# adrelino/mv-lm-icp

Measured on AMD Instinct MI355X. Metric: ICP iterations/sec (NN+Jacobian+LM), higher is better.
Workload: dtype f64; 1 GPU; cfg4: multiview 32 views x 200k pts, point-to-plane, SophusSE3 (E=62); views=32, pts_per_view=200000, edges=62, parallelism=single GPU, nn=auto

## Files before the change

include/mvicp.h:

```cpp
#ifndef MVICP_H
#define MVICP_H

#include <stddef.h>
#include <stdint.h>

#ifdef __cplusplus
extern "C" {
#endif

typedef struct mvicp_ctx mvicp_ctx;

enum mvicp_status {
  MVICP_OK = 0,
  MVICP_ERR_ARG = -1,
  MVICP_ERR_HIP = -2,
  MVICP_ERR_STATE = -3,
  MVICP_ERR_COMM = -4,
  MVICP_ERR_NUMERIC = -5,
  MVICP_ERR_INTERNAL = -6
};

enum mvicp_param {
  MVICP_PARAM_EIGEN_QUATERNION = 0,
  MVICP_PARAM_ANGLE_AXIS = 1,
// ... 33 lines not shown
  long long n, kept;
  int q_exp;
  int has_normals;
  unsigned long long s1, s2_hi, s2_lo;
  double T;
  double threshold;
} mvicp_outlier_stats;
long long mvicp_outlier_filter(mvicp_ctx* ctx, int frame, int k, double std_ratio, double radius, mvicp_outlier_stats* stats);
int mvicp_outlier_fetch(mvicp_ctx* ctx, long long cap_kept, double* xyz, double* nrm, int* idx, long long cap_n, double* mdist, double* kd2);
int mvicp_outlier_threshold(long long n, unsigned long long s1, unsigned long long s2_hi, unsigned long long s2_lo, double std_ratio, double* T);

long long mvicp_knn_search(mvicp_ctx* ctx, int frame, const double* queries, long long m, int k, double radius);
int mvicp_knn_fetch(mvicp_ctx* ctx, long long cap_rows, long long cap_entries, int* cnt, long long* off, int* idx, double* d2);

long long mvicp_fpfh(mvicp_ctx* ctx, int frame, double radius, int max_nn);
int mvicp_fpfh_fetch(mvicp_ctx* ctx, long long cap_rows, double* desc, int* used);

long long mvicp_iss_keypoints(mvicp_ctx* ctx, int frame, double salient_radius, double non_max_radius, double gamma21, double gamma32,
                              int min_neighbors);
int mvicp_iss_fetch(mvicp_ctx* ctx, long long cap_keys, int* idx, double* xyz, double* nrm, long long cap_n, double* saliency, int* cnt_salient,
                    int* cnt_nms);

long long mvicp_estimate_normals(mvicp_ctx* ctx, int frame, int max_nn, double radius, const double* viewpoint);
int mvicp_normals_fetch(mvicp_ctx* ctx, long long cap_rows, double* nrm, double* curvature, int* used);
int mvicp_normals_adopt(mvicp_ctx* ctx);

long long mvicp_fit_normals(mvicp_ctx* ctx, int frame, int max_nn, double radius, const double* viewpoint, int degree);
int mvicp_normals_fit_fetch(mvicp_ctx* ctx, long long cap_rows, unsigned char* fitted);

typedef enum { MVICP_ORIENT_ANCHOR = 0, MVICP_ORIENT_VIEWPOINT = 1, MVICP_ORIENT_DIRECTION = 2 } mvicp_orient_mode;
long long mvicp_orient_normals(mvicp_ctx* ctx, int frame, int source, int k, double radius, int mode, const double* ref3);
int mvicp_orient_fetch(mvicp_ctx* ctx, long long cap_rows, double* nrm, unsigned char* flip, int* comp);
int mvicp_orient_adopt(mvicp_ctx* ctx);

int mvicp_normal_agreement(mvicp_ctx* ctx, const double* poses, int* pos, int* neg);
int mvicp_signs_from_agreement(int n_frames, int n_edges, const int* src, const int* dst, const int* pos, const int* neg, int min_count,
                               unsigned char* flip, int* component);
int mvicp_negate_normals(mvicp_ctx* ctx, int frame);

long long mvicp_feature_match(mvicp_ctx* ctx, const double* a, long long m, const double* b, long long n, int dim);
int mvicp_feature_match_fetch(mvicp_ctx* ctx, long long cap_m, long long cap_n, int* fwd_idx, double* fwd_d2, int* bwd_idx, double* bwd_d2);

long long mvicp_match_pairs(long long m, long long n, const int* fwd_idx, const double* fwd_d2, const int* bwd_idx, int mutual, double ratio,
                            int* pairs);

typedef struct mvicp_consensus_result {
  int best, count, accepted, reserved;
  double pose[16];
} mvicp_consensus_result;
int mvicp_consensus(mvicp_ctx* ctx, const double* p, const double* q, long long n_pairs, long long hypotheses, unsigned long long seed,
                    double tau, double edge_sim, mvicp_consensus_result* result);
int mvicp_consensus_fetch(mvicp_ctx* ctx, long long cap_h, int* count, long long cap_c, unsigned char* flags);

typedef struct mvicp_coarse_edge {
  int pairs, best, count, accepted;
  double pose[16];
} mvicp_coarse_edge;
long long mvicp_coarse_pairs(mvicp_ctx* ctx, const double* desc, const double* xyz, const long long* offsets, int n_sets, int dim, int n_edges,
                             const int* src, const int* dst, const unsigned long long* seeds, int mutual, double ratio, long long hypotheses,
                             double tau, double edge_sim, mvicp_coarse_edge* results);
int mvicp_coarse_pairs_fetch(mvicp_ctx* ctx, int edge, long long cap_pairs, int* pairs, unsigned char* flags);

int mvicp_poses_from_pairs(int n_frames, int n_edges, const int* src, const int* dst, const int* count, const double* pose, int min_count,
                           int root, const double* root_pose, double* poses_out, int* parent, int* parent_edge, int* component);

int mvicp_cache_allowance(const double* pose_src_old, const double* pose_dst_old, const double* pose_src, const double* pose_dst,
                          double max_norm, double* out);

int mvicp_graph_from_overlap(int n_frames, const int* samples, const int* hits, const long long* sumq, int knn, double min_fraction,
                             int skip_frame0, int cap, int* src, int* dst, int* n_components);

int mvicp_set_shard(mvicp_ctx* ctx, int rank, int world);
int mvicp_edge_owner(int n_edges, const int* n_src, int world, int* owner);
int mvicp_comm_unique_id(const char* librccl_path, void* unique_id_128);
int mvicp_comm_init(mvicp_ctx* ctx, const char* librccl_path, const void* unique_id_128, int rank, int world);
int mvicp_comm_nranks(mvicp_ctx* ctx);

typedef int (*mvicp_allreduce_fn)(void* user, double* host_buf, size_t n);
int mvicp_comm_set_callback(mvicp_ctx* ctx, mvicp_allreduce_fn fn, void* user);

int mvicp_correspond(mvicp_ctx* ctx, const double* poses, const unsigned char* fixed, float thresh, int nn_method,
                     int* counts, float* weights);
int mvicp_reset_history(mvicp_ctx* ctx);
int mvicp_get_correspondences(mvicp_ctx* ctx, int edge, int cap, int* first, int* second, double* dist);
typedef struct mvicp_corr { int first; int second; double dist; } mvicp_corr;
int mvicp_map_correspondences(mvicp_ctx* ctx, const mvicp_corr** triples, const long long** offsets);
int mvicp_map_correspondences_async(mvicp_ctx* ctx, const mvicp_corr** triples, const long long** offsets);
int mvicp_wait_correspondences(mvicp_ctx* ctx, int edge);
int mvicp_correspondence_epochs(mvicp_ctx* ctx, const unsigned long long** epochs);
int mvicp_set_correspondences(mvicp_ctx* ctx, int edge, int n, const int* first, const int* second, float weight);

int mvicp_nn_query(mvicp_ctx* ctx, int frame, const double* queries, int n, int nn_method, int* idx, double* d2);

#define MVICP_EDGE_BLOCK 91
int mvicp_linearize(mvicp_ctx* ctx, const double* poses, int point_to_plane, int robust, double* out);
int mvicp_linearize_pair(mvicp_ctx* ctx, const double* poses_a, const double* poses_b, int point_to_plane, int robust, double* out_a, double* out_b);

typedef enum { MVICP_METRIC_POINT = 0, MVICP_METRIC_PLANE = 1, MVICP_METRIC_SYMMETRIC = 2 } mvicp_metric;
int mvicp_linearize_metric(mvicp_ctx* ctx, const double* poses, int metric, int robust, double* out);

int mvicp_linearize_gicp(mvicp_ctx* ctx, const double* poses, double epsilon, int robust, double* out);

typedef struct mvicp_summary {
  double initial_cost, final_cost;
  int iterations;
  int successful_steps;
  int termination;
  int evaluations;
} mvicp_summary;
int mvicp_optimize(mvicp_ctx* ctx, double* poses, unsigned char* fixed, int param, int point_to_plane, int robust,
                   int max_iterations , mvicp_summary* summary);
int mvicp_optimize_metric(mvicp_ctx* ctx, double* poses, unsigned char* fixed, int param, int metric, int robust,
                          int max_iterations, mvicp_summary* summary);
int mvicp_optimize_gicp(mvicp_ctx* ctx, double* poses, unsigned char* fixed, int param, double epsilon, int robust,
                        int max_iterations, mvicp_summary* summary);

typedef int (*mvicp_eval_fn)(void* user, const double* poses, double* blocks);
int mvicp_lm_solve(int n_frames, int n_edges, const int* src, const int* dst, double* poses, unsigned char* fixed, int param,
                   int max_iterations, mvicp_eval_fn eval, void* user, mvicp_summary* summary);

int mvicp_closedform_point_to_point(const double* src, const double* dst, int n, double* pose_out);
int mvicp_closedform_point_to_plane(const double* src, const double* dst, const double* nor, int n, double* pose_out);

int mvicp_set_option(mvicp_ctx* ctx, const char* name, double value);
int mvicp_nn_census(mvicp_ctx* ctx, double* out5);
int mvicp_nn_census_ex(mvicp_ctx* ctx, double* out, int cap);
const char* mvicp_last_nn_launch(mvicp_ctx* ctx);

int mvicp_profile_enable(mvicp_ctx* ctx, int on);
int mvicp_profile_reset(mvicp_ctx* ctx);
int mvicp_profile_get(mvicp_ctx* ctx, const char* kernel, double* total_ms, long long* launches, double* alg_bytes);
int mvicp_profile_get_ex(mvicp_ctx* ctx, const char* kernel, double* out, int cap);
void* mvicp_stream(mvicp_ctx* ctx);
int mvicp_sync(mvicp_ctx* ctx);

#ifdef __cplusplus
}
#endif
#endif
```

mv-lm-icp_amd/csrc/api.cpp:

```cpp
#include <algorithm>
#include <cmath>
#include <cstdlib>
#include <cstring>
#include <ctime>
#include <chrono>
#include <condition_variable>
#include <exception>
#include <limits>
#include <mutex>
#include <new>
#include <thread>

#include "common.h"
#include "comm.h"
#include "nn_tie.h"
#include "../host/se3.h"

namespace mvicp {

static thread_local char g_err[1024] = "";

void set_error(const char* fmt, ...) {
  va_list ap;
  va_start(ap, fmt);
// ... 44 lines not shown
    MV_HIP(hipMalloc((void**)&c->d_scratch, c->scratch_bytes));
  }
  void* d = c->d_scratch + c->scratch_used;
  MV_HIP(hipMemcpyAsync(d, src, bytes, hipMemcpyHostToDevice, c->stream));
  MV_HIP(hipStreamSynchronize(c->stream));
  c->scratch_used += aligned;
  *dptr = d;
  return MVICP_OK;
}

ProfScope::ProfScope(mvicp_ctx* ctx, const char* nm, double bytes) : c(ctx), name(nm), on(ctx->profile) {
  if (on && ctx->profile_level >= 2 && ((std::strncmp(nm, "nn_", 3) != 0 && std::strncmp(nm, "linearize", 9) != 0 && std::strcmp(nm, "comm") != 0) ||
                                        std::strcmp(nm, "nn_tie") == 0)) on = false;
  if (!on) return;
  ProfEntry& pe = c->prof[name];
  auto get = [&]() {
    hipEvent_t ev = nullptr;
    if (!pe.pool.empty()) { ev = pe.pool.back(); pe.pool.pop_back(); }
    else if (hipEventCreate(&ev) != hipSuccess) ev = nullptr;
    return ev;
  };
  a = get(); b = get();
  pe.bytes += bytes;
  if (std::strncmp(nm, "nn_", 3) == 0) { pe.survey_bytes += bytes; pe.queries += bytes / 36.0; }
  pe.launches += 1;
  if (a) (void)hipEventRecord(a, c->stream);
}
ProfScope::~ProfScope() {
  if (!on) return;
  if (b) (void)hipEventRecord(b, c->stream);
  if (a && b) c->prof[name].pending.push_back(std::make_pair(a, b));
}
static double now_ms() {
  timespec ts;
  clock_gettime(CLOCK_MONOTONIC, &ts);
  return ts.tv_sec * 1e3 + ts.tv_nsec * 1e-6;
}
HostScope::HostScope(mvicp_ctx* ctx, const char* nm) : c(ctx), name(nm), t0(0.0), on(ctx->profile) { if (on) t0 = now_ms(); }
HostScope::~HostScope() {
  if (!on) return;
  ProfEntry& pe = c->prof[name];
  pe.ms += now_ms() - t0;
  pe.launches += 1;
}
void prof_collect_lazy(mvicp_ctx* c) {
  for (auto& kv : c->prof) if (kv.second.pending.size() > 256) { prof_collect(c); return; }
}
void prof_collect(mvicp_ctx* c) {
  for (auto& kv : c->prof) {
    ProfEntry& pe = kv.second;
    for (auto& pr : pe.pending) {
      float ms = 0.f;
      if (hipEventSynchronize(pr.second) == hipSuccess && hipEventElapsedTime(&ms, pr.first, pr.second) == hipSuccess) pe.ms += ms;
      pe.pool.push_back(pr.first);
      pe.pool.push_back(pr.second);
    }
    pe.pending.clear();
  }
}

namespace {

template <typename T> int dev_alloc(T** p, size_t n) {
  *p = nullptr;
  if (n == 0) n = 1;
  MV_HIP(hipMalloc((void**)p, sizeof(T) * n));
  return MVICP_OK;
}
template <typename T> void dev_free(T*& p) {
  if (p) (void)hipFree(p);
  p = nullptr;
}

void free_graph(mvicp_ctx* c) {
  dev_free(c->d_esrc); dev_free(c->d_edst); dev_free(c->d_cap_off); dev_free(c->d_count);
  dev_free(c->d_ctl); c->d_nsrc = nullptr; c->d_a = nullptr; c->d_xf = nullptr; c->d_rel = nullptr; c->d_rel2 = nullptr; c->d_dirty = nullptr;
  dev_free(c->d_nn_idx); dev_free(c->d_nn_d2); dev_free(c->d_nn_lb); dev_free(c->d_first); dev_free(c->d_second);
  dev_free(c->d_sblock_off); dev_free(c->d_sel_keys1); c->n_sblocks = 0;
  dev_free(c->d_cd2); dev_free(c->d_qpos); dev_free(c->d_dirty_slots); dev_free(c->d_dslot_off); dev_free(c->d_stream); dev_free(c->d_cblock_off); dev_free(c->d_cblock_cnt);
  dev_free(c->d_sel_hist); dev_free(c->d_median); dev_free(c->d_chunk_edge); dev_free(c->d_chunk_start);
  dev_free(c->d_chunk_first); dev_free(c->d_partials); dev_free(c->d_out);
  c->sym_lo_pin.release(); c->sym_lo_dev.release();
  if (c->h_pin) (void)hipHostFree(c->h_pin);
  c->h_pin = nullptr; c->h_pin_doubles = 0; c->d_res_host = nullptr; c->d_blocks_host = nullptr; c->lin_out = nullptr;
  c->census_pending = false; c->spec_ready = false; c->spec2_ready = false; c->spec_arm = false; c->d_spec_host = nullptr; c->d_adev_host = nullptr; c->d_res_target = nullptr; c->d_a_check = nullptr;
  dev_free(c->d_xblock_cnt); c->export_valid = false; c->export_in_flight = false; c->export_chunks = 0;
  for (hipEvent_t ev : c->export_events) (void)hipEventDestroy(ev);
  c->export_events.clear();
  if (c->d_export) (void)hipFree(c->d_export);
  if (c->h_export) (void)hipHostFree(c->h_export);
  c->d_export = nullptr; c->h_export = nullptr; c->export_cap = 0;
  c->E = 0; c->total_cap = 0; c->n_cblocks = 0; c->n_chunks = 0; c->hist.have_corr = false;
}

int bind(mvicp_ctx* c) {
  if (!c) { set_error("null context"); return MVICP_ERR_ARG; }
  MV_HIP(hipSetDevice(c->device));
  return MVICP_OK;
}

int ensure_pin(mvicp_ctx* c, size_t doubles) {
  if (doubles <= c->h_pin_doubles) return MVICP_OK;
  if (c->h_pin) MV_HIP(hipHostFree(c->h_pin));
  c->h_pin = nullptr;
  MV_HIP(hipHostMalloc((void**)&c->h_pin, sizeof(double) * doubles, hipHostMallocMapped));
  std::memset(c->h_pin, 0, sizeof(double) * doubles);
  c->h_pin_doubles = doubles;
  return MVICP_OK;
}

}

static void fill_rel_into(mvicp_ctx* c, const double* poses, double* h);
void fill_rel(mvicp_ctx* c, const double* poses) {
  fill_rel_into(c, poses, c->h_pin + c->ctl_r2_off);
}
static void fill_rel_into(mvicp_ctx* c, const double* poses, double* h) {
  for (int e = 0; e < c->E; ++e) {
    const double* Ps = poses + 16 * (size_t)c->esrc[e];
    const double* Pd = poses + 16 * (size_t)c->edst[e];
    double* r = h + (size_t)e * kEdgeRel;
    for (int j = 0; j < 3; ++j)
      for (int i = 0; i < 3; ++i) r[i + 3 * j] = Pd[0 + 4 * i] * Ps[0 + 4 * j] + Pd[1 + 4 * i] * Ps[1 + 4 * j] + Pd[2 + 4 * i] * Ps[2 + 4 * j];
    const double dt[3] = {Ps[12] - Pd[12], Ps[13] - Pd[13], Ps[14] - Pd[14]};
    for (int i = 0; i < 3; ++i) r[9 + i] = Pd[0 + 4 * i] * dt[0] + Pd[1 + 4 * i] * dt[1] + Pd[2 + 4 * i] * dt[2];
  }
}
int upload_rel(mvicp_ctx* c, const double* poses) {
  fill_rel(c, poses);
  MV_HIP(hipMemcpyAsync(c->d_rel, c->h_pin + c->ctl_r2_off, sizeof(double) * c->ctl_r2, hipMemcpyHostToDevice, c->stream));
  return MVICP_OK;
}

static void fill_rel_sym(mvicp_ctx* c, const double* poses, double* h, double* lo) {
  typedef long double ld;
  for (int e = 0; e < c->E; ++e) {
    const double* Ps = poses + 16 * (size_t)c->esrc[e];
    const double* Pd = poses + 16 * (size_t)c->edst[e];
    ld M[3][3];
    for (int i = 0; i < 3; ++i) for (int j = 0; j < 3; ++j) M[i][j] = Pd[i + 4 * j];
    ld C[3][3];
    C[0][0] = M[1][1] * M[2][2] - M[1][2] * M[2][1]; C[0][1] = M[1][2] * M[2][0] - M[1][0] * M[2][2]; C[0][2] = M[1][0] * M[2][1] - M[1][1] * M[2][0];
    C[1][0] = M[0][2] * M[2][1] - M[0][1] * M[2][2]; C[1][1] = M[0][0] * M[2][2] - M[0][2] * M[2][0]; C[1][2] = M[0][1] * M[2][0] - M[0][0] * M[2][1];
    C[2][0] = M[0][1] * M[1][2] - M[0][2] * M[1][1]; C[2][1] = M[0][2] * M[1][0] - M[0][0] * M[1][2]; C[2][2] = M[0][0] * M[1][1] - M[0][1] * M[1][0];
    ld det = M[0][0] * C[0][0] + M[0][1] * C[0][1] + M[0][2] * C[0][2];
    if (!(det > 0.5L && det < 2.0L)) {
      for (int i = 0; i < 3; ++i) for (int j = 0; j < 3; ++j) C[i][j] = M[i][j];
      det = 1.0L;
    }
    ld v[kEdgeRel];
    const ld dt[3] = {(ld)Ps[12] - (ld)Pd[12], (ld)Ps[13] - (ld)Pd[13], (ld)Ps[14] - (ld)Pd[14]};
    for (int i = 0; i < 3; ++i) {
      const ld inv_i[3] = {C[0][i] / det, C[1][i] / det, C[2][i] / det};
      for (int j = 0; j < 3; ++j) v[i + 3 * j] = inv_i[0] * (ld)Ps[0 + 4 * j] + inv_i[1] * (ld)Ps[1 + 4 * j] + inv_i[2] * (ld)Ps[2 + 4 * j];
      v[9 + i] = inv_i[0] * dt[0] + inv_i[1] * dt[1] + inv_i[2] * dt[2];
    }
    for (int k = 0; k < kEdgeRel; ++k) {
      const double hi = (double)v[k];
      h[(size_t)e * kEdgeRel + k] = hi;
      lo[(size_t)e * kEdgeRel + k] = (double)(v[k] - (ld)hi);
    }
  }
}
int upload_rel_sym(mvicp_ctx* c, const double* poses) {
  const size_t bytes = sizeof(double) * (size_t)c->E * kEdgeRel;
  MV_CHECK(c->sym_lo_pin.reserve(bytes));
  MV_CHECK(c->sym_lo_dev.reserve(bytes));
// ... 1247 lines not shown
    chunk_edge.swap(ce); chunk_start.swap(cs);
  }
  const size_t cap = (size_t)c->total_cap;
  MV_CHECK(dev_alloc(&c->d_esrc, E)); MV_CHECK(dev_alloc(&c->d_edst, E)); MV_CHECK(dev_alloc(&c->d_cap_off, E + 1));
  MV_CHECK(dev_alloc(&c->d_count, E));
  c->ctl_r1 = (size_t)E * kEdgeXf + (size_t)E + 2 * (size_t)E;
  c->ctl_rel2_off = (c->ctl_r1 + 1) & ~(size_t)1;
  c->ctl_r2_off = c->ctl_rel2_off + (size_t)E * kEdgeRel;
  c->ctl_r2 = (size_t)E * (kEdgeRel + 1);
  MV_CHECK(dev_alloc(&c->d_ctl, c->ctl_r2_off + c->ctl_r2));
  MV_HIP(hipMemset(c->d_ctl, 0, sizeof(double) * std::max<size_t>(c->ctl_r2_off + c->ctl_r2, 1)));
  c->d_xf = c->d_ctl; c->d_nsrc = reinterpret_cast<int*>(c->d_ctl + (size_t)E * kEdgeXf); c->d_dirty = c->d_nsrc + E;
  c->d_sel_lohi = c->d_ctl + (size_t)E * (kEdgeXf + 1);
  c->d_rel = c->d_ctl + c->ctl_r2_off; c->d_a = c->d_rel + (size_t)E * kEdgeRel; c->d_rel2 = c->d_ctl + c->ctl_rel2_off;
  MV_CHECK(dev_alloc(&c->d_nn_idx, cap)); MV_CHECK(dev_alloc(&c->d_nn_d2, cap)); MV_CHECK(dev_alloc(&c->d_nn_lb, cap));
  MV_CHECK(dev_alloc(&c->d_first, cap)); MV_CHECK(dev_alloc(&c->d_second, cap)); MV_CHECK(dev_alloc(&c->d_cd2, cap));
  MV_CHECK(dev_alloc(&c->d_stream, 10 * cap));
  MV_CHECK(dev_alloc(&c->d_qpos, cap));
  MV_HIP(hipMemset(c->d_qpos, 0xff, sizeof(int) * std::max<size_t>(cap, 1)));
  c->export_valid = false; c->export_off.assign((size_t)E + 1, 0);
  c->corr_epoch.assign(E, 0);
  for (int e = 0; e < E; ++e) c->corr_epoch[e] = ++c->epoch_counter;
  c->dslot_off.assign(E + 1, 0);
  for (int e = 0; e < E; ++e) c->dslot_off[e + 1] = c->dslot_off[e] + (int)(((c->owned[e] ? c->frames[src[e]].n : 0) + 255) / 256);
  c->n_dslots = c->dslot_off[E];
  MV_CHECK(dev_alloc(&c->d_dirty_slots, (size_t)c->n_dslots)); MV_CHECK(dev_alloc(&c->d_dslot_off, (size_t)E + 1));
  MV_HIP(hipMemset(c->d_dirty_slots, 0, sizeof(int) * std::max<size_t>((size_t)c->n_dslots, 1)));
  MV_HIP(hipMemcpy(c->d_dslot_off, c->dslot_off.data(), sizeof(int) * (E + 1), hipMemcpyHostToDevice));
  MV_CHECK(dev_alloc(&c->d_cblock_off, E + 1)); MV_CHECK(dev_alloc(&c->d_cblock_cnt, (size_t)c->n_cblocks));
  MV_CHECK(dev_alloc(&c->d_sel_hist, (size_t)E * (2048 + 2)));
  MV_HIP(hipMemset(c->d_sel_hist, 0, sizeof(unsigned int) * std::max<size_t>((size_t)E * (2048 + 2), 1)));
  c->sel_scratch_clean = true;
  c->sblock_off.assign(E + 1, 0);
  for (int e = 0; e < E; ++e) c->sblock_off[e + 1] = c->sblock_off[e] + (int)(((c->owned[e] ? c->frames[src[e]].n : 0) + kSelBlock - 1) / kSelBlock);
  c->n_sblocks = c->sblock_off[E];
  MV_CHECK(dev_alloc(&c->d_sblock_off, (size_t)E + 1));
  MV_HIP(hipMemcpy(c->d_sblock_off, c->sblock_off.data(), sizeof(int) * (E + 1), hipMemcpyHostToDevice));
  MV_CHECK(dev_alloc(&c->d_sel_keys1, cap));
  if (cap > c->far_cap) {
    if (c->d_far_list) MV_HIP(hipFree(c->d_far_list));
    c->d_far_list = nullptr; c->far_cap = 0;
    MV_HIP(hipMalloc(&c->d_far_list, sizeof(int) * 2 * cap));
    c->far_cap = cap;
  }
  MV_CHECK(warm_nn_grid(c)); MV_CHECK(warm_nn_tile(c)); MV_CHECK(warm_nn_mfma(c));
  if (c->opt.tie_rule && !(c->opt.tie_lazy && c->world == 1)) {
    std::vector<int> need;
    for (int e = 0; e < E; ++e) if (c->owned[e]) need.push_back(dst[e]);
    MV_CHECK(ensure_tie_trees(c, need));
  }
  MV_CHECK(dev_alloc(&c->d_median, E));
  MV_CHECK(dev_alloc(&c->d_chunk_edge, (size_t)c->n_chunks)); MV_CHECK(dev_alloc(&c->d_chunk_start, (size_t)c->n_chunks));
  MV_CHECK(dev_alloc(&c->d_chunk_first, E + 1));
  MV_CHECK(dev_alloc(&c->d_partials, 2 * (size_t)c->n_chunks * kLinPartial));
  MV_CHECK(dev_alloc(&c->d_out, (size_t)E * (MVICP_EDGE_BLOCK + 3) + 2));
  MV_HIP(hipMemset(c->d_out, 0, sizeof(double) * ((size_t)E * (MVICP_EDGE_BLOCK + 3) + 2)));
  if (E) {
    MV_HIP(hipMemcpy(c->d_esrc, src, sizeof(int) * E, hipMemcpyHostToDevice));
    MV_HIP(hipMemcpy(c->d_edst, dst, sizeof(int) * E, hipMemcpyHostToDevice));
    MV_HIP(hipMemset(c->d_count, 0, sizeof(int) * E));
  }
  MV_HIP(hipMemcpy(c->d_cap_off, c->cap_off.data(), sizeof(long long) * (E + 1), hipMemcpyHostToDevice));
  MV_HIP(hipMemcpy(c->d_cblock_off, c->cblock_off.data(), sizeof(int) * (E + 1), hipMemcpyHostToDevice));
  MV_HIP(hipMemcpy(c->d_chunk_first, c->chunk_first.data(), sizeof(int) * (E + 1), hipMemcpyHostToDevice));
  if (c->n_chunks) {
    MV_HIP(hipMemcpy(c->d_chunk_edge, chunk_edge.data(), sizeof(int) * c->n_chunks, hipMemcpyHostToDevice));
    MV_HIP(hipMemcpy(c->d_chunk_start, chunk_start.data(), sizeof(int) * c->n_chunks, hipMemcpyHostToDevice));
  }
  c->pin_blocks_off = c->ctl_r2_off + c->ctl_r2;
  c->pin_res_off = c->pin_blocks_off + (size_t)E * MVICP_EDGE_BLOCK;
  c->pin_misc_off = c->pin_res_off + 2 * (size_t)E + 2;
  c->pin_spec_off = c->pin_misc_off + 4 * (size_t)E + 64;
  c->pin_adev_off = c->pin_spec_off + (size_t)E * (MVICP_EDGE_BLOCK + 3) + 2;
  if (c->h_pin) { MV_HIP(hipHostFree(c->h_pin)); c->h_pin = nullptr; c->h_pin_doubles = 0; }
  c->pin_spec2_off = (c->pin_adev_off + (size_t)E + 8 + 1) & ~(size_t)1;
  c->pin_rel2_off = c->pin_spec2_off + (size_t)E * MVICP_EDGE_BLOCK + ((size_t)E * MVICP_EDGE_BLOCK & 1);
  c->pin_blocks2_off = (c->pin_rel2_off + (size_t)E * kEdgeRel + 1) & ~(size_t)1;
  MV_CHECK(ensure_pin(c, c->pin_blocks2_off + (size_t)E * MVICP_EDGE_BLOCK + 8));
  {
    void* dp = nullptr;
    MV_HIP(hipHostGetDevicePointer(&dp, c->h_pin, 0));
    c->d_blocks_host = (double*)dp + c->pin_blocks_off;
    c->d_res_host = (double*)dp + c->pin_res_off;
    c->d_spec_host = (double*)dp + c->pin_spec_off;
    c->d_adev_host = (double*)dp + c->pin_adev_off;
    c->d_spec2_host = (double*)dp + c->pin_spec2_off;
    c->d_blocks2_host = (double*)dp + c->pin_blocks2_off;
  }
  c->spec_ready = false; c->spec_arm = false;
  c->spec2_ready = false; c->spec2_armed = false;
  if (!c->h_census) MV_HIP(hipHostMalloc((void**)&c->h_census, 8 * sizeof(unsigned long long), hipHostMallocDefault));
  return MVICP_OK;
} MVICP_GUARD_ABI

static void forget_history(mvicp_ctx* c) {
  c->hist.forget(c->E);
  c->export_valid = false;
  for (int e = 0; e < c->E; ++e) c->corr_epoch[e] = ++c->epoch_counter;
  c->spec_ready = false; c->spec_arm = false;
  c->spec2_ready = false; c->spec2_armed = false;
}

int mvicp_reset_history(mvicp_ctx* c) try {
  MV_CHECK(bind(c));
  MV_HIP(hipStreamSynchronize(c->stream));
  forget_history(c);
  return MVICP_OK;
} MVICP_GUARD_ABI

static int correspond_once(mvicp_ctx* c, const double* poses, const unsigned char* fixed, float thresh, int nn_method, int* counts, float* weights, bool* tie_unresolved);

int mvicp_correspond(mvicp_ctx* c, const double* poses, const unsigned char* fixed, float thresh, int nn_method, int* counts, float* weights) try {
  MV_CHECK(bind(c));
  struct Forget { mvicp_ctx* c; bool ok = false; ~Forget() { if (!ok) { (void)hipStreamSynchronize(c->stream); forget_history(c); } } } forget{c};
  bool unresolved = false;
  MV_CHECK(correspond_once(c, poses, fixed, thresh, nn_method, counts, weights, &unresolved));
  if (!unresolved) { forget.ok = true; return MVICP_OK; }
  std::vector<int> need;
  for (int e = 0; e < c->E; ++e) if (c->active[e] && !c->frames[c->edst[e]].has_tie) need.push_back(c->edst[e]);
  MV_HIP(hipStreamSynchronize(c->stream));
  MV_CHECK(ensure_tie_trees(c, need));
  forget_history(c);
  unresolved = false;
  MV_CHECK(correspond_once(c, poses, fixed, thresh, nn_method, counts, weights, &unresolved));
  if (unresolved) { set_error("tie fix-up still without a tree after building them"); return MVICP_ERR_INTERNAL; }
  forget.ok = true;
  return MVICP_OK;
} MVICP_GUARD_ABI


namespace {
struct CorrMarks {
  mvicp_ctx* c; double t;
  void operator()(const char* nm) { if (c->profile) { const double now = now_ms(); ProfEntry& pe = c->prof[nm]; pe.ms += now - t; pe.launches += 1; t = now; } }
};
size_t out_blocks(const mvicp_ctx* c) { return (size_t)c->E * MVICP_EDGE_BLOCK; }
size_t out_tail(const mvicp_ctx* c) { return 3 * (size_t)c->E + 1; }
size_t out_armed(const mvicp_ctx* c) { return out_blocks(c) + 2 * (size_t)c->E; }
void spec_failed(mvicp_ctx* c) { c->hist.spec_flags_valid = false; c->spec_arm = false; }
}

static SearchInputs search_inputs(mvicp_ctx* c, const double* poses, const unsigned char* fixed, float thresh, int nn_method) {
  c->plan_frames.resize(c->frames.size());
  for (size_t k = 0; k < c->frames.size(); ++k) {
    const FrameDev& f = c->frames[k];
    PlanFrame& pf = c->plan_frames[k];
    pf.n = f.n; pf.max_norm = f.max_norm; pf.cell = f.grid.cell; pf.has_grid = f.has_grid; pf.has_tie = f.has_tie; pf.has_snor = f.grid.snor != nullptr;
  }
  SearchInputs in;
  in.E = c->E; in.n_frames = c->n_frames;
  in.esrc = c->esrc.data(); in.edst = c->edst.data(); in.owned = c->owned.data(); in.frames = c->plan_frames.data();
  in.poses = poses; in.fixed = fixed; in.thresh = thresh; in.nn_method = nn_method;
  in.exchange = c->comm != nullptr || c->ar_fn != nullptr; in.world = c->world;
  return in;
}

static size_t stage_queued_evaluations(mvicp_ctx* c, const SearchPlan& plan, const double* poses) {
  if (!plan.spec_arm) return c->ctl_r1;
  c->spec_poses.resize(16 * (size_t)c->n_frames);
  double xp[7];
  for (int k = 0; k < c->n_frames; ++k) { se3::pose_to_x(c->hist.spec_param, poses + 16 * (size_t)k, xp); se3::x_to_pose(c->hist.spec_param, xp, &c->spec_poses[16 * (size_t)k]); }
  fill_rel(c, c->spec_poses.data());
  c->spec_q_plane = c->hist.spec_plane; c->spec_q_robust = c->hist.spec_robust;
  if (plan.spec2_plan && c->opt.lin_pair) fill_rel_into(c, c->hist.last_cand_poses.data(), c->h_pin + c->ctl_rel2_off);
  return c->ctl_r2_off + (size_t)c->E * kEdgeRel;
}

static int launch_local_search(mvicp_ctx* c, const SearchInputs& in, const SearchPlan& plan, double bound, size_t upload_doubles, CorrMarks& mark) {
  MV_HIP(hipMemcpyAsync(c->d_ctl, c->h_pin, sizeof(double) * upload_doubles, hipMemcpyHostToDevice, c->stream));
  if (c->fault_inject > 0 && --c->fault_inject == 0) { set_error("injected launch failure (option fault_inject)"); return MVICP_ERR_HIP; }
  if (plan.method == MVICP_NN_BRUTE) MV_CHECK(launch_nn_brute_edges(c));
  else if (plan.method == MVICP_NN_GRID) MV_CHECK(launch_nn_grid_edges(c, bound, plan));
  else {
    if (c->profile && plan.eps_over_mu >= 0.0) { ProfEntry& pe = c->prof["auto.eps_over_mu"]; pe.ms = plan.eps_over_mu; pe.launches += 1; }
    MV_CHECK(launch_nn_tile_edges(c, bound, plan));
  }
  record_queued(in, c->opt, plan, c->hist);
  if (!plan.all_unchanged) c->export_valid = false;
  mark("host.corr.nn_launch");
  if (!plan.nothing_can_change) {
    MV_CHECK(launch_compact(c, bound));
    MV_CHECK(launch_gather_stream(c));
  }
  if (plan.sel_skip) { c->h_pin[c->pin_res_off + 2 * (size_t)c->E] = plan.spec_arm ? 1.0 : 0.0; return MVICP_OK; }
  return plan.use_bracket ? launch_select_bracket(c) : launch_select_median(c, bound);
}

static int queue_exchanged_evaluation(mvicp_ctx* c, const SearchPlan& plan) {
  c->lin_out = c->d_out;
  if (plan.spec_arm) return launch_linearize(c, c->spec_q_plane, c->spec_q_robust);
  if (hipMemsetAsync(c->d_out, 0, sizeof(double) * out_blocks(c), c->stream) != hipSuccess ||
      hipMemsetAsync(c->d_out + out_armed(c) + 1, 0, sizeof(double) * (size_t)c->E, c->stream) != hipSuccess) { set_error("hipMemsetAsync of the exchange buffer failed"); return MVICP_ERR_HIP; }
  return MVICP_OK;
}

static int queue_evaluations(mvicp_ctx* c, const SearchPlan& plan) {
  auto second_armed = [c]() { c->spec2_armed = true; c->spec2_poses = c->hist.last_cand_poses; c->spec2_plane = c->spec_q_plane; c->spec2_robust = c->spec_q_robust; };
  c->spec2_armed = false;
  if (plan.spec2_plan && c->opt.lin_pair) {
    const int st = launch_linearize_pair(c, c->spec_q_plane, c->spec_q_robust, c->d_spec_host, c->d_spec2_host);
    if (st == MVICP_OK) second_armed();
    return st;
  }
  c->lin_out = c->d_spec_host;
  int st = launch_linearize(c, c->spec_q_plane, c->spec_q_robust);
  if (st == MVICP_OK && plan.spec2_plan) {
    fill_rel_into(c, c->hist.last_cand_poses.data(), c->h_pin + c->pin_rel2_off);
    if (hipMemcpyAsync(c->d_rel, c->h_pin + c->pin_rel2_off, sizeof(double) * (size_t)c->E * kEdgeRel, hipMemcpyHostToDevice, c->stream) == hipSuccess) {
      c->lin_out = c->d_spec2_host;
      st = launch_linearize(c, c->spec_q_plane, c->spec_q_robust);
      if (st == MVICP_OK) second_armed();
    }
  }
  return st;
}

static int exchange_out(mvicp_ctx* c, size_t off, size_t len, const char* what, int st_local, char* local_msg, bool* entered) {
  *entered = true;
  if (st_local != MVICP_OK) {
    std::memcpy(local_msg, g_err, sizeof(g_err));
    if (hipMemsetAsync(c->d_out + out_armed(c), 0xFF, sizeof(double), c->stream) != hipSuccess) {
      if (off == 0) set_error("%s — and the exchange buffer could not be poisoned: the peers of this rank will block in the collective", local_msg);
      *entered = false;
      return st_local;
    }
  }
  int st;
  { ProfScope pc(c, "comm", 8.0 * (double)len); st = comm_allreduce_sum(c, c->d_out + off, len); }
  if (st == MVICP_OK && hipMemcpyAsync(c->h_pin + c->pin_spec_off + off, c->d_out + off, sizeof(double) * len, hipMemcpyDeviceToHost, c->stream) != hipSuccess) {
    set_error("hipMemcpyAsync of the exchanged %s failed", what); st = MVICP_ERR_HIP;
  }
  return st;
}

static int redo_select(mvicp_ctx* c, double bound, bool exchange, char* local_msg) {
  int st = launch_select_median(c, bound);
  if (exchange) {
    const int st_r = st;
    bool entered;
    st = exchange_out(c, out_blocks(c), out_tail(c), "tail", st_r, local_msg, &entered);
    if (!entered) { spec_failed(c); return st_r; }
    if (st == MVICP_OK) st = stream_wait(c);
    if (st != MVICP_OK) { spec_failed(c); return st; }
    if (std::isnan(c->h_pin[c->pin_spec_off + out_armed(c)])) {
      forget_history(c);
      if (st_r != MVICP_OK) { set_error("%s", local_msg); return st_r; }
      set_error("a peer rank failed before the second exchange of this search (poisoned exchange buffer); cross-round state dropped on every rank");
      return MVICP_ERR_COMM;
    }
    return MVICP_OK;
  }
// ... 36 lines not shown
    if (!entered) { spec_failed(c); return st_local; }
  } else if (plan.spec_arm) st_q = queue_evaluations(c, plan);
  mark("host.corr.post_launch");
  if (st_q == MVICP_OK) st_q = stream_wait(c);
  if (st_q != MVICP_OK) { spec_failed(c); return st_q; }
  if (in.exchange && std::isnan(c->h_pin[c->pin_spec_off + armed])) {
    forget_history(c);
    c->census_pending = false;
    if (st_local != MVICP_OK) { set_error("%s", local_msg); return st_local; }
    set_error("a peer rank failed before the exchange of this search (poisoned exchange buffer); nothing was updated, cross-round state dropped on every rank");
    return MVICP_ERR_COMM;
  }
  census_resolve(c);
  if (plan.tie_launched && c->h_tie_seen && c->h_tie_seen[1] != 0u) *tie_unresolved = true;
  if (plan.tie_launched && c->h_tie_seen && c->h_tie_seen[2] != 0u) { set_error("tie fix-up: a walk ran out of stack (a tree deeper than its recorded levels)"); return MVICP_ERR_INTERNAL; }
  mark("host.corr.wait");
  const double* hr = in.exchange ? c->h_pin + c->pin_spec_off + nb : c->h_pin + c->pin_res_off;
  bool redone = false;
  for (int e = 0; e < E; ++e) if (hr[2 * e + 1] < 0.0) redone = true;
  if (redone) MV_CHECK(redo_select(c, bound, in.exchange, local_msg));
  c->spec_ready = record_arrived(in, plan, c->hist, c->h_tie_seen ? *c->h_tie_seen : 1u, c->h_far_seen ? *c->h_far_seen : 1u, hr,
                                 in.exchange ? hr + 2 * (size_t)E + 1 : c->h_pin + c->pin_adev_off, redone);
  c->spec2_ready = c->spec_ready && c->spec2_armed;
  c->spec2_armed = false;
  c->spec_arm = false;
  double* ha = c->h_pin + c->ctl_r2_off + (size_t)E * kEdgeRel;
  for (int e = 0; e < E; ++e) {
    ha[e] = (double)c->hist.h_weight[e];
    if (counts) counts[e] = c->hist.h_count[e];
    if (weights) weights[e] = c->hist.h_weight[e];
    if (!plan.unchanged[e]) c->corr_epoch[e] = ++c->epoch_counter;
  }
  mark("host.corr.finish");
  if (c->profile) prof_collect_lazy(c);
  guard.ok = true;
  return MVICP_OK;
}

static int ensure_export(mvicp_ctx* c, bool wait = true) {
  if (!c->export_valid) {
    HostScope hs(c, "host.export");
    MV_CHECK(launch_export(c));
    c->export_valid = true;
  }
  if (wait && c->export_in_flight) {
    MV_CHECK(stream_wait(c));
    c->export_in_flight = false;
    if (c->profile) prof_collect_lazy(c);
  }
  return MVICP_OK;
}

int mvicp_map_correspondences(mvicp_ctx* c, const mvicp_corr** triples, const long long** offsets) try {
  MV_CHECK(bind(c));
  if (!triples || !offsets) { set_error("null output"); return MVICP_ERR_ARG; }
  if (!c->hist.have_corr) { set_error("no correspondences yet"); return MVICP_ERR_STATE; }
  MV_CHECK(ensure_export(c));
  *triples = (const mvicp_corr*)c->h_export;
  *offsets = c->export_off.data();
  return MVICP_OK;
} MVICP_GUARD_ABI

int mvicp_map_correspondences_async(mvicp_ctx* c, const mvicp_corr** triples, const long long** offsets) try {
  MV_CHECK(bind(c));
  if (!triples || !offsets) { set_error("null output"); return MVICP_ERR_ARG; }
  if (!c->hist.have_corr) { set_error("no correspondences yet"); return MVICP_ERR_STATE; }
  MV_CHECK(ensure_export(c, false));
  *triples = (const mvicp_corr*)c->h_export;
  *offsets = c->export_off.data();
  return MVICP_OK;
} MVICP_GUARD_ABI

int mvicp_wait_correspondences(mvicp_ctx* c, int edge) try {
  MV_CHECK(bind(c));
  if (edge < 0 || edge >= c->E) { set_error("edge %d out of range", edge); return MVICP_ERR_ARG; }
  if (!c->export_valid) { set_error("no export in flight: call mvicp_map_correspondences_async after the search"); return MVICP_ERR_STATE; }
  if (!c->export_in_flight || c->export_chunks == 0) return MVICP_OK;
  const int k = c->export_edge_chunk[edge];
  MV_HIP(hipEventSynchronize(c->export_events[k]));
  if (k == c->export_chunks - 1) c->export_in_flight = false;
  return MVICP_OK;
} MVICP_GUARD_ABI

int mvicp_correspondence_epochs(mvicp_ctx* c, const unsigned long long** epochs) try {
  MV_CHECK(bind(c));
  if (!epochs) { set_error("null output"); return MVICP_ERR_ARG; }
  if (c->E == 0) { set_error("no graph"); return MVICP_ERR_STATE; }
  *epochs = c->corr_epoch.data();
  return MVICP_OK;
} MVICP_GUARD_ABI

int mvicp_get_correspondences(mvicp_ctx* c, int edge, int cap, int* first, int* second, double* dist) try {
  MV_CHECK(bind(c));
  if (edge < 0 || edge >= c->E) { set_error("edge %d out of range", edge); return MVICP_ERR_ARG; }
  if (!c->hist.have_corr) { set_error("no correspondences yet"); return MVICP_ERR_STATE; }
  if (!c->owned[edge]) { set_error("edge %d is owned by another rank", edge); return MVICP_ERR_STATE; }
  const int n = c->hist.h_count[edge];
  if (cap < n) { set_error("capacity %d < count %d", cap, n); return MVICP_ERR_ARG; }
  if (!c->hist.explicit_list[edge]) {
    if (n == 0) return 0;
    MV_CHECK(ensure_export(c));
    const mvicp_corr* t = (const mvicp_corr*)c->h_export + c->export_off[edge];
    if (c->export_off[edge + 1] - c->export_off[edge] != n) { set_error("export of edge %d holds %lld triples, expected %d", edge, c->export_off[edge + 1] - c->export_off[edge], n); return MVICP_ERR_STATE; }
    for (int i = 0; i < n; ++i) {
      if (first) first[i] = t[i].first;
      if (second) second[i] = t[i].second;
      if (dist) dist[i] = t[i].dist;
    }
    return n;
  }
  const size_t off = (size_t)c->cap_off[edge];
  MV_HIP(hipStreamSynchronize(c->stream));
  std::vector<int> a(n), b(n);
  std::vector<double> d(n);
  if (n) {
    MV_HIP(hipMemcpy(a.data(), c->d_first + off, sizeof(int) * n, hipMemcpyDeviceToHost));
    MV_HIP(hipMemcpy(b.data(), c->d_second + off, sizeof(int) * n, hipMemcpyDeviceToHost));
    MV_HIP(hipMemcpy(d.data(), c->d_cd2 + off, sizeof(double) * n, hipMemcpyDeviceToHost));
  }
  const std::vector<int>& so = c->frames[c->esrc[edge]].grid.h_order;
  const std::vector<int>& dorder = c->frames[c->edst[edge]].grid.h_order;
  std::vector<int> perm(n);
  for (int i = 0; i < n; ++i) { a[i] = so[a[i]]; b[i] = dorder[b[i]]; perm[i] = i; }
  std::stable_sort(perm.begin(), perm.end(), [&](int x, int y) { return a[x] < a[y]; });
  for (int i = 0; i < n; ++i) {
    const int k = perm[i];
    if (first) first[i] = a[k];
    if (second) second[i] = b[k];
    if (dist) dist[i] = std::sqrt(d[k]);
  }
  return n;
} MVICP_GUARD_ABI

int mvicp_set_correspondences(mvicp_ctx* c, int edge, int n, const int* first, const int* second, float weight) try {
  MV_CHECK(bind(c));
  if (edge < 0 || edge >= c->E) { set_error("edge %d out of range", edge); return MVICP_ERR_ARG; }
  if (!c->owned[edge]) { set_error("edge %d is owned by another rank", edge); return MVICP_ERR_STATE; }
  const int ns = c->frames[c->esrc[edge]].n, nd = c->frames[c->edst[edge]].n;
  if (n < 0 || n > ns) { set_error("n=%d exceeds the edge capacity N_src=%d", n, ns); return MVICP_ERR_ARG; }
  if (n > 0 && (!first || !second)) { set_error("null correspondence list (n=%d)", n); return MVICP_ERR_ARG; }
  for (int i = 0; i < n; ++i)
    if (first[i] < 0 || first[i] >= ns || second[i] < 0 || second[i] >= nd) { set_error("correspondence %d out of range", i); return MVICP_ERR_ARG; }
  const size_t off = (size_t)c->cap_off[edge];
  MV_HIP(hipStreamSynchronize(c->stream));
  if (n) {
    const std::vector<int>& si = c->frames[c->esrc[edge]].grid.h_inv;
    const std::vector<int>& di = c->frames[c->edst[edge]].grid.h_inv;
    std::vector<int> a(n), b(n);
    for (int i = 0; i < n; ++i) { a[i] = si[first[i]]; b[i] = di[second[i]]; }
    MV_HIP(hipMemcpy(c->d_first + off, a.data(), sizeof(int) * n, hipMemcpyHostToDevice));
    MV_HIP(hipMemcpy(c->d_second + off, b.data(), sizeof(int) * n, hipMemcpyHostToDevice));
    MV_HIP(hipMemset(c->d_cd2 + off, 0, sizeof(double) * n));
  }
  c->hist.explicit_edge(edge, n, weight);
  c->spec_ready = false; c->spec2_ready = false;
  c->export_valid = false;
  c->corr_epoch[edge] = ++c->epoch_counter;
  const double a = (double)weight;
  MV_HIP(hipMemcpy(c->d_count + edge, &n, sizeof(int), hipMemcpyHostToDevice));
  {
    const int not_identity = -1;
    MV_HIP(hipMemcpy(c->d_nsrc + edge, &not_identity, sizeof(int), hipMemcpyHostToDevice));
  }
  MV_HIP(hipMemcpy(c->d_a + edge, &a, sizeof(double), hipMemcpyHostToDevice));
  c->h_pin[c->ctl_r2_off + (size_t)c->E * kEdgeRel + edge] = a;
  const int one = 1;
// ... 8 lines not shown
  if (frame < 0 || frame >= c->n_frames) { set_error("frame %d out of range", frame); return MVICP_ERR_ARG; }
  if (n < 0 || (n && (!queries || !idx || !d2))) { set_error("bad query buffers"); return MVICP_ERR_ARG; }
  if (nn_method < MVICP_NN_AUTO || nn_method > MVICP_NN_TILE) { set_error("unknown nn_method %d", nn_method); return MVICP_ERR_ARG; }
  MV_CHECK(finish_builds(c));
  const FrameDev& f = c->frames[frame];
  if (f.n == 0) { set_error("frame %d is empty (nanoflann throws here: nanoflann.hpp:904)", frame); return MVICP_ERR_STATE; }
  if (n == 0) return MVICP_OK;
  double* dq = nullptr; int* di = nullptr; double* dd = nullptr;
  MV_CHECK(dev_alloc(&dq, 3 * (size_t)n)); MV_CHECK(dev_alloc(&di, (size_t)n)); MV_CHECK(dev_alloc(&dd, (size_t)n));
  MV_HIP(hipMemcpy(dq, queries, sizeof(double) * 3 * (size_t)n, hipMemcpyHostToDevice));
  int method = (nn_method == MVICP_NN_AUTO || nn_method == MVICP_NN_TILE) ? MVICP_NN_GRID : nn_method;
  if (c->opt.tie_rule) MV_CHECK(ensure_tie_trees(c, std::vector<int>(1, frame)));
  if (method == MVICP_NN_GRID && !f.has_grid) method = MVICP_NN_BRUTE;
  int st;
  if (method == MVICP_NN_BRUTE) st = launch_nn_brute_queries(c, f, dq, n, di, dd);
  else if (method == MVICP_NN_GRID) st = launch_nn_grid_queries(c, f, dq, n, di, dd);
  else { set_error("unknown nn_method %d", nn_method); st = MVICP_ERR_ARG; }
  if (st == MVICP_OK) {
    hipError_t e1 = hipStreamSynchronize(c->stream);
    if (e1 == hipSuccess) census_resolve(c);
    if (e1 == hipSuccess && c->opt.tie_rule && c->h_tie_seen && c->h_tie_seen[2] != 0u) { set_error("tie fix-up: a walk ran out of stack (a tree deeper than its recorded levels)"); st = MVICP_ERR_INTERNAL; }
    hipError_t e2 = hipMemcpy(idx, di, sizeof(int) * n, hipMemcpyDeviceToHost);
    hipError_t e3 = hipMemcpy(d2, dd, sizeof(double) * n, hipMemcpyDeviceToHost);
    if (e1 != hipSuccess || e2 != hipSuccess || e3 != hipSuccess) { set_error("nn_query copy-back failed"); st = MVICP_ERR_HIP; }
  }
  dev_free(dq); dev_free(di); dev_free(dd);
  if (c->profile) prof_collect_lazy(c);
  return st;
} MVICP_GUARD_ABI

int mvicp_linearize(mvicp_ctx* c, const double* poses, int point_to_plane, int robust, double* out) try {
  MV_CHECK(bind(c));
  if (!poses || !out) { set_error("null argument"); return MVICP_ERR_ARG; }
  if (c->E == 0) { set_error("no graph"); return MVICP_ERR_STATE; }
  MV_CHECK(evaluate_blocks(c, poses, point_to_plane ? MVICP_METRIC_PLANE : MVICP_METRIC_POINT, robust, out));
  if (c->profile) prof_collect_lazy(c);
  return MVICP_OK;
} MVICP_GUARD_ABI

int mvicp_linearize_metric(mvicp_ctx* c, const double* poses, int metric, int robust, double* out) try {
  if (metric != MVICP_METRIC_POINT && metric != MVICP_METRIC_PLANE && metric != MVICP_METRIC_SYMMETRIC) { set_error("metric %d is not an mvicp_metric", metric); return MVICP_ERR_ARG; }
  MV_CHECK(bind(c));
  if (!poses || !out) { set_error("null argument"); return MVICP_ERR_ARG; }
  if (c->E == 0) { set_error("no graph"); return MVICP_ERR_STATE; }
  MV_CHECK(evaluate_blocks(c, poses, metric, robust, out));
  if (c->profile) prof_collect_lazy(c);
  return MVICP_OK;
} MVICP_GUARD_ABI

int mvicp_linearize_gicp(mvicp_ctx* c, const double* poses, double epsilon, int robust, double* out) try {
  if (!gicp_epsilon_ok(epsilon)) { set_error("gicp epsilon %g is not within [1e-6, 1]", epsilon); return MVICP_ERR_ARG; }
  MV_CHECK(bind(c));
  if (!poses || !out) { set_error("null argument"); return MVICP_ERR_ARG; }
  if (c->E == 0) { set_error("no graph"); return MVICP_ERR_STATE; }
  c->gicp_eps = epsilon;
  MV_CHECK(evaluate_blocks(c, poses, kMetricGicp, robust, out));
  if (c->profile) prof_collect_lazy(c);
  return MVICP_OK;
} MVICP_GUARD_ABI

int mvicp_linearize_pair(mvicp_ctx* c, const double* poses_a, const double* poses_b, int point_to_plane, int robust, double* out_a, double* out_b) try {
  MV_CHECK(bind(c));
  if (!poses_a || !poses_b || !out_a || !out_b) { set_error("null argument"); return MVICP_ERR_ARG; }
  if (c->E == 0) { set_error("no graph"); return MVICP_ERR_STATE; }
  if (c->comm || c->ar_fn) {
    MV_CHECK(evaluate_blocks(c, poses_a, point_to_plane ? MVICP_METRIC_PLANE : MVICP_METRIC_POINT, robust, out_a));
    MV_CHECK(evaluate_blocks(c, poses_b, point_to_plane ? MVICP_METRIC_PLANE : MVICP_METRIC_POINT, robust, out_b));
  } else {
    MV_CHECK(evaluate_pair(c, poses_a, poses_b, point_to_plane ? MVICP_METRIC_PLANE : MVICP_METRIC_POINT, robust, out_a, out_b));
  }
  if (c->profile) prof_collect_lazy(c);
  return MVICP_OK;
} MVICP_GUARD_ABI

int mvicp_set_option(mvicp_ctx* c, const char* name, double value) try {
  MV_CHECK(bind(c));
  if (!name) { set_error("null option name"); return MVICP_ERR_ARG; }
  if (std::strcmp(name, "async_build") == 0) { c->async_build = value != 0.0; return MVICP_OK; }
  if (std::strcmp(name, "grid_target") == 0 || std::strcmp(name, "grid_curve") == 0) MV_CHECK(finish_builds(c));
  if (std::strcmp(name, "nn_tree_only") == 0) { c->opt.nn_tree_only = value != 0.0; return MVICP_OK; }
  if (std::strcmp(name, "nn_cache") == 0) { c->opt.nn_cache_enable = value != 0.0; c->hist.nn_cache_valid = false; return MVICP_OK; }
  if (std::strcmp(name, "lin_chunk") == 0) { c->lin_chunk_override = (int)value; return MVICP_OK; }
  if (std::strcmp(name, "list_reuse") == 0) { c->opt.list_reuse = value != 0.0; return MVICP_OK; }
  if (std::strcmp(name, "lin_interleave") == 0) { c->lin_interleave = value != 0.0; return MVICP_OK; }
  if (std::strcmp(name, "lin_share_p") == 0) { c->lin_share_p = value != 0.0; return MVICP_OK; }
  if (std::strcmp(name, "lin_pair") == 0) { c->opt.lin_pair = value != 0.0; return MVICP_OK; }
  if (std::strcmp(name, "nn_census") == 0) { c->nn_census = value != 0.0; return MVICP_OK; }
  if (std::strcmp(name, "nn_skip_far") == 0) { c->opt.nn_skip_far = value != 0.0; return MVICP_OK; }
  if (std::strcmp(name, "sel_bracket") == 0) { c->opt.sel_bracket = value != 0.0; return MVICP_OK; }
  if (std::strcmp(name, "sel_reuse") == 0) { c->opt.sel_reuse = value != 0.0; return MVICP_OK; }
  if (std::strcmp(name, "prune_rho") == 0) { c->prune_rho = value; return MVICP_OK; }
  if (std::strcmp(name, "grid_curve") == 0) { c->grid_curve = (int)value; return MVICP_OK; }
  if (std::strcmp(name, "auto_settle") == 0) { c->opt.auto_settle = value; return MVICP_OK; }
  if (std::strcmp(name, "auto_switch") == 0) { c->opt.auto_switch = value; return MVICP_OK; }
  if (std::strcmp(name, "nn_cell") == 0) { c->opt.nn_cell = value != 0.0; return MVICP_OK; }
  if (std::strcmp(name, "nn_search_factor") == 0) { if (!(value >= 0.0)) { set_error("nn_search_factor < 0"); return MVICP_ERR_ARG; } c->nn_search_factor = value; c->hist.nn_cache_valid = false; return MVICP_OK; }
  if (std::strcmp(name, "tie_rule") == 0) {
    const bool on = value != 0.0;
    if (on != c->opt.tie_rule) { MV_HIP(hipStreamSynchronize(c->stream)); c->opt.tie_rule = on; forget_history(c); }
    return MVICP_OK;
  }
  if (std::strcmp(name, "tie_lazy") == 0) { c->opt.tie_lazy = value != 0.0; return MVICP_OK; }
  if (std::strcmp(name, "tile_seed") == 0) { c->tile_seed = value != 0.0; return MVICP_OK; }
  if (std::strcmp(name, "tile_bounds") == 0) { c->opt.tile_bounds = (int)value; return MVICP_OK; }
  if (std::strcmp(name, "tile_mu") == 0) { if (!(value > 0.0 && value <= 1.0)) { set_error("tile_mu outside (0, 1]"); return MVICP_ERR_ARG; } c->opt.tile_mu = value; return MVICP_OK; }
  if (std::strcmp(name, "mfma_kacc") == 0) { if (!(value >= 1.0 && value <= 1024.0)) { set_error("mfma_kacc outside [1, 1024]"); return MVICP_ERR_ARG; } c->mfma_kacc = value; return MVICP_OK; }
  if (std::strcmp(name, "mfma_lbt") == 0) { c->mfma_lbt = (int)value; return MVICP_OK; }
  if (std::strcmp(name, "mfma_entry") == 0) { c->mfma_entry = (int)value; return MVICP_OK; }
  if (std::strcmp(name, "mfma_trig") == 0) { c->mfma_trig = (int)value; return MVICP_OK; }
  if (std::strcmp(name, "tile_mfma") == 0) { c->opt.tile_mfma = (int)value; return MVICP_OK; }
  if (std::strcmp(name, "tile_waves") == 0) { c->tile_waves = (int)value; return MVICP_OK; }
  if (std::strcmp(name, "cache_mfma_ratio") == 0) { c->opt.cache_mfma_ratio = value; return MVICP_OK; }
  if (std::strcmp(name, "reject_cache") == 0) { c->reject_cache = value != 0.0; return MVICP_OK; }
  if (std::strcmp(name, "tile_miss") == 0) { if (!(value >= 0.0 && value <= 64.0)) { set_error("tile_miss outside [0, 64]"); return MVICP_ERR_ARG; } c->tile_miss = (int)value; return MVICP_OK; }
  if (std::strcmp(name, "tile_cache") == 0) { c->opt.tile_cache = (int)value; return MVICP_OK; }
  if (std::strcmp(name, "voxel_permute") == 0) { c->voxel_permute = value != 0.0; return MVICP_OK; }
  if (std::strcmp(name, "knn_order") == 0) { c->knn_order = value != 0.0; return MVICP_OK; }
  if (std::strcmp(name, "match_chunk") == 0) {
    if (!(value >= 1.0 && value < 2147483648.0)) { set_error("match_chunk must be in [1, 2^31)"); return MVICP_ERR_ARG; }
    c->match_chunk = (int)value; return MVICP_OK;
  }
  if (std::strcmp(name, "spin_wait") == 0) { c->spin_wait = value != 0.0; return MVICP_OK; }
  if (std::strcmp(name, "fault_inject") == 0) { c->fault_inject = (int)value; return MVICP_OK; }
  if (std::strcmp(name, "fault_inject_build") == 0) { c->fault_inject_build.store((int)value); return MVICP_OK; }
  if (std::strcmp(name, "fault_inject_eval") == 0) { c->fault_inject_eval = (int)value; return MVICP_OK; }
  if (std::strcmp(name, "spec_eval") == 0) { c->opt.spec_enable = value != 0.0; c->spec_ready = false; c->spec2_ready = false; return MVICP_OK; }
  if (std::strcmp(name, "spec2_eval") == 0) { c->opt.spec2_enable = value != 0.0; c->spec2_ready = false; return MVICP_OK; }
  if (std::strcmp(name, "grid_target") == 0) {
    if (!(value >= 0.5 && value <= 64.0)) { set_error("grid_target out of range"); return MVICP_ERR_ARG; }
    c->grid_target = value;
    return MVICP_OK;
  }
  set_error("unknown option '%s'", name);
  return MVICP_ERR_ARG;
} MVICP_GUARD_ABI
int mvicp_nn_census_ex(mvicp_ctx* c, double* out, int cap) try {
  MV_CHECK(bind(c));
  if (!out || cap < 0) { set_error("bad output buffer"); return MVICP_ERR_ARG; }
  const double v[10] = {c->nn_queries, c->nn_candidates, c->nn_nodes, c->nn_far, c->nn_hits, c->nn_fetched, c->nn_dbg[0], c->nn_dbg[1], c->nn_dbg[2], c->nn_dbg[3]};
  const int n = std::min(cap, 10);
  for (int i = 0; i < n; ++i) out[i] = v[i];
  return n;
} MVICP_GUARD_ABI
const char* mvicp_last_nn_launch(mvicp_ctx* c) { return c ? c->last_nn_launch : ""; }
int mvicp_nn_census(mvicp_ctx* c, double* out5) try {
  const int n = mvicp_nn_census_ex(c, out5, 5);
  return n < 0 ? n : MVICP_OK;
} MVICP_GUARD_ABI

int mvicp_profile_enable(mvicp_ctx* c, int on) try {
  MV_CHECK(bind(c));
  c->profile = on != 0;
  c->profile_level = on;
  return MVICP_OK;
} MVICP_GUARD_ABI
int mvicp_profile_reset(mvicp_ctx* c) try {
  MV_CHECK(bind(c));
  MV_HIP(hipStreamSynchronize(c->stream));
  prof_collect(c);
  for (auto& kv : c->prof) { kv.second.ms = 0; kv.second.launches = 0; kv.second.bytes = 0; kv.second.survey_bytes = 0; kv.second.queries = 0; }
  c->nn_candidates = c->nn_nodes = c->nn_far = c->nn_queries = c->nn_hits = c->nn_fetched = 0;
  for (int k = 0; k < 4; ++k) c->nn_dbg[k] = 0;
  return MVICP_OK;
} MVICP_GUARD_ABI
static void prof_sum(mvicp_ctx* c, const char* kernel, double out[5]) {
  for (int k = 0; k < 5; ++k) out[k] = 0.0;
// ... 39 lines not shown
```

mv-lm-icp_amd/csrc/common.h:

```cpp
#pragma once
#include <hip/hip_runtime.h>

#include <atomic>
#include <cstdarg>
#include <cstdio>
#include <future>
#include <map>
#include <memory>
#include <string>
#include <vector>

#include "../../include/mvicp.h"
#include "abi_guard.h"
#include "search_plan.h"

namespace mvicp {

void set_error(const char* fmt, ...);

#define MV_HIP(expr)                                                                          \
  do {                                                                                        \
    hipError_t _e = (expr);                                                                   \
    if (_e != hipSuccess) {                                                                   \
      mvicp::set_error("%s:%d: %s -> %s", __FILE__, __LINE__, #expr, hipGetErrorString(_e));  \
// ... 129 lines not shown
  void release() { dev.release(); *this = FpfhStage(); }
};
struct MatchStage {
  DevBuf dev, tmp;
  int* fwd_idx = nullptr; int* bwd_idx = nullptr; double* fwd_d2 = nullptr; double* bwd_d2 = nullptr;
  long long m = -1, n = -1;
  void release() { dev.release(); tmp.release(); *this = MatchStage(); }
};
struct ConsensusStage {
  DevBuf dev;
  int* count = nullptr; unsigned char* flags = nullptr;
  long long H = -1, c = -1;
  void release() { dev.release(); *this = ConsensusStage(); }
};
struct CoarseStage {
  DevBuf dev, tmp, work;
  int* pairs = nullptr; unsigned char* flags = nullptr;
  std::vector<long long> seg; std::vector<int> cnt;
  int edges = -1;
  void release() { dev.release(); tmp.release(); work.release(); *this = CoarseStage(); }
};
struct IssStage {
  DevBuf dev, tmp; PinBuf pin;
  double* sal = nullptr; int* cnt_s = nullptr; int* cnt_n = nullptr; int* idx = nullptr; double* xyz = nullptr; double* nrm = nullptr;
  long long n = -1, k = 0; int has_normals = 0;
  void release() { dev.release(); tmp.release(); pin.release(); *this = IssStage(); }
};
struct NormalsStage {
  DevBuf dev;
  double* nrm = nullptr; double* curv = nullptr; int* used = nullptr; unsigned char* fitted = nullptr;
  long long rows = -1; int frame = -1, has_fit = 0;
  void drop_result() { rows = -1; frame = -1; has_fit = 0; }
  void release() { dev.release(); *this = NormalsStage(); }
};

struct OrientStage {
  DevBuf dev; PinBuf pin;
  double* nrm = nullptr; unsigned char* flip = nullptr; int* comp = nullptr;
  long long rows = -1, comps = 0; int frame = -1;
  void drop_result() { rows = -1; comps = 0; frame = -1; }
  void release() { dev.release(); pin.release(); *this = OrientStage(); }
};
struct AgreementStage {
  DevBuf dev; PinBuf pin;
  void release() { dev.release(); pin.release(); *this = AgreementStage(); }
};

struct RcclApi;

}

struct mvicp_ctx {
  int device = 0;
  hipStream_t stream = nullptr;
  int n_frames = 0;
  std::vector<mvicp::FrameDev> frames;

  mvicp::SearchOptions opt;
  mvicp::SearchHistory hist;
  mvicp::SearchPlan plan;
  std::vector<mvicp::PlanFrame> plan_frames;

  int rank = 0, world = 1;
  int E = 0;
  std::vector<int> esrc, edst;
  std::vector<char> owned;
  std::vector<long long> cap_off;
  long long total_cap = 0;

  double* d_ctl = nullptr; size_t ctl_r1 = 0, ctl_rel2_off = 0, ctl_r2_off = 0, ctl_r2 = 0;
  int* d_esrc = nullptr; int* d_edst = nullptr;
  long long* d_cap_off = nullptr;
  int* d_nsrc = nullptr;
  int* d_count = nullptr;
  double* d_a = nullptr;
  double* d_xf = nullptr;
  double* d_rel = nullptr;
  double* d_rel2 = nullptr;
  int* d_nn_idx = nullptr; double* d_nn_d2 = nullptr;
  float* d_nn_lb = nullptr;
  int* d_first = nullptr; int* d_second = nullptr; double* d_cd2 = nullptr;
  int* d_qpos = nullptr;
  int* d_dirty = nullptr;
  int* d_dirty_slots = nullptr; int* d_dslot_off = nullptr; std::vector<int> dslot_off; int n_dslots = 0;
  void* d_export = nullptr; void* h_export = nullptr; size_t export_cap = 0;
  int* d_xblock_cnt = nullptr;
  std::vector<long long> export_off;
  bool export_valid = false;
  std::vector<hipEvent_t> export_events; std::vector<int> export_edge_chunk; int export_chunks = 0; bool export_in_flight = false;
  std::vector<unsigned long long> corr_epoch;
  unsigned long long epoch_counter = 0;
  double* d_stream = nullptr;
  int n_cblocks = 0;
  std::vector<int> cblock_off;
  int* d_cblock_off = nullptr; int* d_cblock_cnt = nullptr;
  unsigned int* d_sel_hist = nullptr;
  double* d_median = nullptr;
  int n_sblocks = 0; std::vector<int> sblock_off; int* d_sblock_off = nullptr;
  double* d_sel_lohi = nullptr;
  bool sel_scratch_clean = false;
  double* d_sel_keys1 = nullptr;
  bool lin_interleave = true;
  bool lin_share_p = true;
  int lin_chunk_override = 0;
  int lin_chunk = 4096;
  int n_chunks = 0;
  std::vector<int> chunk_first;
  int* d_chunk_edge = nullptr; int* d_chunk_start = nullptr; int* d_chunk_first = nullptr;
  double* d_partials = nullptr;
  double gicp_eps = 1e-3;
  mvicp::PinBuf sym_lo_pin; mvicp::DevBuf sym_lo_dev;
  double* d_out = nullptr;
  double* d_res_target = nullptr;
  double* h_pin = nullptr; size_t h_pin_doubles = 0;
  size_t pin_blocks_off = 0, pin_res_off = 0, pin_misc_off = 0;
  double* d_res_host = nullptr;
  double* d_blocks_host = nullptr;
  double* lin_out = nullptr;
  int spec_q_plane = 0, spec_q_robust = 0;
  bool spec_arm = false;
  bool spec_ready = false;
  std::vector<double> spec_poses;
  size_t pin_spec_off = 0, pin_adev_off = 0; double* d_spec_host = nullptr; double* d_adev_host = nullptr;
  bool spec2_armed = false, spec2_ready = false; int spec2_plane = 0, spec2_robust = 0;
  std::vector<double> spec2_poses;
  size_t pin_spec2_off = 0, pin_rel2_off = 0; double* d_spec2_host = nullptr;
  size_t pin_blocks2_off = 0; double* d_blocks2_host = nullptr;
  double* d_a_check = nullptr;
  bool spin_wait = false;
  unsigned long long* h_census = nullptr;
  bool census_pending = false; double census_nq = 0; int census_kind = 0; const char* census_scope = "nn_grid";
  int* d_split_idx = nullptr; double* d_split_d2 = nullptr; size_t split_cap = 0;

  char* ov_dev = nullptr; char* ov_pin = nullptr; size_t ov_bytes = 0;

  mvicp::VoxelStage vox;
  int voxel_permute = 1;
  mvicp::OutlierStage out;
  mvicp::KnnStage knn;
  int knn_order = 1;
  mvicp::FpfhStage fpfh;
  mvicp::MatchStage match;
  int match_chunk = 2048;
  mvicp::ConsensusStage cons;
  mvicp::CoarseStage coarse;
  mvicp::IssStage iss;
  mvicp::NormalsStage nrm;
  mvicp::OrientStage ori;
  mvicp::AgreementStage agree;
  std::vector<char> src_fixed;

  struct CachedTable { std::vector<char> bytes; void* d = nullptr; size_t cap = 0; };
  std::map<std::string, CachedTable> tables;
  char* d_scratch = nullptr; size_t scratch_bytes = 0, scratch_used = 0;
  std::vector<char> active;

  mvicp::RcclApi* rccl = nullptr;
  void* comm = nullptr;
  mvicp_allreduce_fn ar_fn = nullptr; void* ar_user = nullptr;
  std::vector<double> ar_host;

  bool async_build = true;
  std::atomic<int> fault_inject_build{0};
  int fault_inject = 0, fault_inject_eval = 0;
  bool nn_census = false;
  void* d_census = nullptr; size_t census_bytes = 0;
// ... 98 lines not shown
```

mv-lm-icp_amd/csrc/nn_cache.h:

```cpp
#pragma once
#include "common.h"
#include "nn_list.h"

namespace mvicp {

__device__ __forceinline__ double cache_eps(const double* sxf, double p0, double p1, double p2) {
  const double e0 = sxf[kXfDM] * p0 + sxf[kXfDM + 3] * p1 + sxf[kXfDM + 6] * p2 + sxf[kXfDv];
  const double e1 = sxf[kXfDM + 1] * p0 + sxf[kXfDM + 4] * p1 + sxf[kXfDM + 7] * p2 + sxf[kXfDv + 1];
  const double e2 = sxf[kXfDM + 2] * p0 + sxf[kXfDM + 5] * p1 + sxf[kXfDM + 8] * p2 + sxf[kXfDv + 2];
  return sqrt(e0 * e0 + e1 * e1 + e2 * e2) * (1.0 + 1e-9) + sxf[kXfCache];
}

__device__ __forceinline__ bool cache_hit(double eps, float lb_old, double d, double bound, bool same_query_hits, bool reject_cache) {
  const double nlb = (double)lb_old - eps;
  const bool still_rejected = eps != 0.0 && d >= bound && nlb > sqrt(bound) * (1.0 + 1e-9);
  return (same_query_hits && eps == 0.0) || sqrt(d) * (1.0 + 1e-12) < nlb || (reject_cache && still_rejected);
}

__device__ __forceinline__ bool cache_still_none(double allowance, const float* out_lb, int i) { return allowance == 0.0 && out_lb[i] == -1.f; }

template <typename Job>
__device__ __forceinline__ void cache_refresh(const Job& job, int i, int pi, double d, double eps, float lb_old, double bound) {
  if (eps != 0.0) {
    job.out_d2[i] = d;
    job.out_lb[i] = __double2float_rd((double)lb_old - eps);
    if (job.list.dirty) update_list_entry(job.list, i, pi, d, bound, true);
  }
}

}
```

mv-lm-icp_amd/csrc/nn_grid.hip:

```cpp
#include <algorithm>
#include <atomic>
#include <cmath>
#include <cstring>
#include <limits>
#include <numeric>
#include <system_error>
#include <thread>
#include <unordered_set>

#include "build_common.h"
#include "common.h"
#include "nn_cache.h"
#include "nn_census.h"
#include "nn_list.h"
#include "nn_metric.h"
#include "nn_tie.h"

namespace mvicp {

namespace {

#ifndef MVICP_GRID_THREADS
#define MVICP_GRID_THREADS 256
#endif
constexpr int NT = MVICP_GRID_THREADS;
constexpr unsigned long long EMPTY = ~0ull;

struct GridView {
  const double* spts; const int* sidx; const PointRec* srec; int n;
  const PointRec* crec;
  const HashEntry* table; unsigned int mask; int shift;
  double ox, oy, oz, h, inv_h;
  int dx, dy, dz;
  const float* oct; int oct_leaf; long long oct_first_leaf;
  const BrickEntry* bricks; const uint2* celltab; int bx, by, bz;
};

struct GridJob {
  GridView dst;
  const double* q; const int* qidx;
  const double* xf;
  int n;
  int* out_idx; double* out_d2;
  const int* inv;
  ListRef list;
  float* out_lb;
  int seed;
  TieRef tie;
};

__device__ __forceinline__ unsigned long long __reduce_add_u64(unsigned long long v) {
  unsigned long long total = 0;
  unsigned long long mask = __ballot(1);
  while (mask) {
    const int l = __ffsll((long long)mask) - 1;
    total += __shfl(v, l, 64);
    mask &= mask - 1;
  }
  return total;
}
__device__ __forceinline__ bool __lane0() {
  const unsigned long long mask = __ballot(1);
  return (int)(threadIdx.x & 63) == __ffsll((long long)mask) - 1;
}

__global__ void dirty_reduce_kernel(int E, const int* __restrict__ slot_off, int* __restrict__ slots, int* __restrict__ dirty) {
  const int e = blockIdx.x;
  int any = 0;
  for (int k = slot_off[e] + threadIdx.x; k < slot_off[e + 1]; k += blockDim.x) {
    const int v = slots[k];
    if (v) { any = 1; slots[k] = 0; }
  }
  if (__syncthreads_or(any) && threadIdx.x == 0) dirty[e] = 1;
}

template <bool TREE_ONLY>
__global__ __launch_bounds__(NT) void nn_grid_kernel(const GridJob* __restrict__ jobs, double bound, double search, unsigned long long* __restrict__ stats, int skip_far,
                                                     int2* __restrict__ far_list, unsigned int* __restrict__ far_count, double prune_rho) {
  __shared__ double sxf[kEdgeXf];
  __shared__ uint2 s_rng[8][NT];
  const GridJob& job = jobs[blockIdx.y];
  const int i = blockIdx.x * NT + threadIdx.x;
  if (blockIdx.x * NT >= job.n) return;
  const bool has_xf = job.xf != nullptr;
  if (has_xf && threadIdx.x < kEdgeXf) sxf[threadIdx.x] = job.xf[threadIdx.x];
  __syncthreads();
  if (i >= job.n) return;
  const GridView& g = job.dst;

  double qx, qy, qz;
  {
    const double p0 = job.q[3 * (size_t)i], p1 = job.q[3 * (size_t)i + 1], p2 = job.q[3 * (size_t)i + 2];
    if (has_xf) xf_point(sxf, p0, p1, p2, qx, qy, qz);
    else { qx = p0; qy = p1; qz = p2; }
  }
  const int out = i;

  double best = search;
  int bi = 0x7fffffff;
  bool resolved = false;
  unsigned int n_cand = 0;
  double second = 1.7976931348623157e308;

  const double slack = has_xf ? sxf[kXfCache] : -1.0;
  double rp2 = -1.0;
  if (!TREE_ONLY && job.seed) {
    const int pi = job.out_idx[out];
    if (pi < 0 && job.out_lb != nullptr && cache_still_none(slack, job.out_lb, out)) {
      if (stats) {
        unsigned long long c1 = __reduce_add_u64(1ull);
        const size_t slot = ((size_t)blockIdx.y * gridDim.x + blockIdx.x) * (NT / 64) + (threadIdx.x >> 6);
        if (__lane0()) atomicAdd(&stats[8 * slot + 3], c1);
      }
      return;
    }
    if (pi >= 0 && pi < g.n) {
      const double* tp = g.spts + 3 * (size_t)pi;
      const double d = dist2(qx, qy, qz, tp[0], tp[1], tp[2]);
      if (slack >= 0.0 && job.out_lb != nullptr) {
        const double p0 = job.q[3 * (size_t)i], p1 = job.q[3 * (size_t)i + 1], p2 = job.q[3 * (size_t)i + 2];
        const double eps = cache_eps(sxf, p0, p1, p2);
        const float lb_old = job.out_lb[out];
        if (cache_hit(eps, lb_old, d, bound, true, false)) {
          cache_refresh(job, out, pi, d, eps, lb_old, bound);
          if (stats) {
            unsigned long long c1 = __reduce_add_u64(1ull);
            const size_t slot = ((size_t)blockIdx.y * gridDim.x + blockIdx.x) * (NT / 64) + (threadIdx.x >> 6);
            if (__lane0()) atomicAdd(&stats[8 * slot + 3], c1);
          }
          return;
        }
      }
      if (prune_rho > 0.0) { const double rp = sqrt(d) + prune_rho * g.h; rp2 = rp * rp * 1.002; }
    }
  }

  double m2 = 0.0;
  double skipped = 1.7976931348623157e308;
  if (!TREE_ONLY) {
    const double cx = (qx - g.ox) * g.inv_h - 0.5, cy = (qy - g.oy) * g.inv_h - 0.5, cz = (qz - g.oz) * g.inv_h - 0.5;
    const double lim = 2.0e6;
    const int bx = (int)floor(fmin(fmax(cx, -lim), lim)), by = (int)floor(fmin(fmax(cy, -lim), lim)), bz = (int)floor(fmin(fmax(cz, -lim), lim));
    unsigned long long key[8];
    unsigned int slot[8];
    HashEntry ent[8];
    const double ax = qx - (g.ox + (bx + 1) * g.h), ay = qy - (g.oy + (by + 1) * g.h), az = qz - (g.oz + (bz + 1) * g.h);
    const double ax2 = ax * ax * 0.998, ay2 = ay * ay * 0.998, az2 = az * az * 0.998;
    const int home = (ax >= 0.0 ? 1 : 0) | (ay >= 0.0 ? 2 : 0) | (az >= 0.0 ? 4 : 0);
#pragma unroll
    for (int c = 0; c < 8; ++c) {
      const int ix = bx + (c & 1), iy = by + ((c >> 1) & 1), iz = bz + (c >> 2);
      bool in = !(ix < 0 || iy < 0 || iz < 0 || ix >= g.dx || iy >= g.dy || iz >= g.dz);
      if (rp2 >= 0.0) {
        const int df = c ^ home;
        const double lbc = ((df & 1) ? ax2 : 0.0) + ((df & 2) ? ay2 : 0.0) + ((df & 4) ? az2 : 0.0);
        if (lbc > rp2) { in = false; skipped = fmin(skipped, lbc); }
      }
      key[c] = in ? cell_key(ix, iy, iz) : EMPTY;
      slot[c] = hash_slot(key[c], g.shift) & g.mask;
    }
#pragma unroll
    for (int c = 0; c < 8; ++c) {
      ent[c].key = EMPTY; ent[c].start = 0; ent[c].count = 0;
      if (key[c] != EMPTY) ent[c] = g.table[slot[c]];
    }
#pragma unroll
    for (int c = 0; c < 8; ++c) {
      while (ent[c].key != key[c] && ent[c].key != EMPTY) {
        slot[c] = (slot[c] + 1) & g.mask;
        ent[c] = g.table[slot[c]];
      }
      if (ent[c].key == EMPTY) ent[c].count = 0;
    }
#pragma unroll
    for (int c = 0; c < 8; ++c) {
      s_rng[c][threadIdx.x] = make_uint2(ent[c].start, ent[c].count);
      n_cand += ent[c].count;
    }
    {
      int c = -1;
      unsigned int j = 0, je = 0;
      for (;;) {
        while (j == je && c < 7) { ++c; const uint2 r = s_rng[c][threadIdx.x]; j = r.x; je = r.x + r.y; }
        if (j == je) break;
        const double2* p = reinterpret_cast<const double2*>(g.crec + j);
        const double2 a = p[0], b = p[1];
        const double d = dist2(qx, qy, qz, a.x, a.y, b.x);
        const int oi = (int)__double_as_longlong(b.y);
        if (d < best || (d == best && oi < bi)) {
          if (bi != 0x7fffffff) second = fmin(second, best);
          best = d; bi = oi;
        } else {
          second = fmin(second, d);
        }
        ++j;
      }
    }
    const double fx = g.ox + bx * g.h, fy = g.oy + by * g.h, fz = g.oz + bz * g.h;
    double m = fmin(fmin(qx - fx, fx + 2.0 * g.h - qx), fmin(fmin(qy - fy, fy + 2.0 * g.h - qy), fmin(qz - fz, fz + 2.0 * g.h - qz)));
    m *= 0.999;
    m2 = m > 0.0 ? m * m : 0.0;
    resolved = (m > 0.0) && (best < m2) && (bi != 0x7fffffff);
  }
  if (!TREE_ONLY && !resolved && bi == 0x7fffffff && job.seed) {
    const int pi = job.out_idx[out];
    if (pi >= 0 && pi < g.n) {
      const double2* tp = reinterpret_cast<const double2*>(g.srec + pi);
      const double2 ta = tp[0], tb = tp[1];
      const double d = dist2(qx, qy, qz, ta.x, ta.y, tb.x);
      if (d < best) { best = d; bi = (int)__double_as_longlong(tb.y); }
    }
  }
  job.out_idx[out] = bi == 0x7fffffff ? -1 : (job.inv ? job.inv[bi] : bi);
  job.out_d2[out] = best;
  if (job.out_lb != nullptr) job.out_lb[out] = resolved ? __double2float_rd(sqrt(fmin(fmin(second, m2), skipped)) * (1.0 - 1e-12)) : 0.f;
  if (job.list.dirty && (resolved || skip_far)) update_list_entry(job.list, i, bi == 0x7fffffff ? -1 : job.inv[bi], best, bound, false);
  if (resolved && bi != 0x7fffffff && second == best) tie_report(job.tie, (unsigned int)i);
  if (!resolved && !skip_far) {
    const unsigned long long mask = __ballot(1);
    const int lane = threadIdx.x & 63;
    const int leader = __ffsll((long long)mask) - 1;
    const int rank = __popcll(mask & ((1ull << lane) - 1ull));
    unsigned int base = 0;
    if (lane == leader) base = atomicAdd(far_count, (unsigned int)__popcll(mask));
    base = __shfl(base, leader, 64);
    far_list[base + rank] = make_int2((int)blockIdx.y, i);
  }
  if (stats) {
    unsigned long long c = n_cand, far = resolved ? 0 : 1;
    c = __reduce_add_u64(c); far = __reduce_add_u64(far);
    const size_t slot = ((size_t)blockIdx.y * gridDim.x + blockIdx.x) * (NT / 64) + (threadIdx.x >> 6);
    if (__lane0()) { atomicAdd(&stats[8 * slot], c); atomicAdd(&stats[8 * slot + 2], far); }
  }
}


constexpr int CELL_HS = 128;
constexpr int CELL_POOL = 960;
constexpr int CELL_SPAN = 6;
constexpr unsigned int CELL_UNSET = 0xfffffffeu, CELL_NOFIT = 0xffffffffu;

__device__ __forceinline__ void wave_sync() {
  __builtin_amdgcn_fence(__ATOMIC_RELEASE, "wavefront");
  __builtin_amdgcn_wave_barrier();
  __builtin_amdgcn_fence(__ATOMIC_ACQUIRE, "wavefront");
}

__device__ __forceinline__ double cell_lb2(const GridView& g, int ix, int iy, int iz, double qx, double qy, double qz, double tol) {
  const double lx = g.ox + ix * g.h, ly = g.oy + iy * g.h, lz = g.oz + iz * g.h;
  const double gx = fmax(fmax(lx - qx, qx - (lx + g.h)) - tol, 0.0);
  const double gy = fmax(fmax(ly - qy, qy - (ly + g.h)) - tol, 0.0);
  const double gz = fmax(fmax(lz - qz, qz - (lz + g.h)) - tol, 0.0);
  return (gx * gx + gy * gy + gz * gz) * 0.999999;
}

__device__ __forceinline__ bool cell_insert(unsigned long long* __restrict__ hk, unsigned long long key) {
  unsigned int s = hash_slot(key, 64 - 7) & (CELL_HS - 1);
  for (int probe = 0; probe < 24; ++probe) {
    const unsigned long long old = atomicCAS(&hk[s], EMPTY, key);
    if (old == EMPTY || old == key) return true;
    s = (s + 1) & (CELL_HS - 1);
  }
  return false;
}
__device__ __forceinline__ int cell_find(const unsigned long long* __restrict__ hk, unsigned long long key) {
  unsigned int s = hash_slot(key, 64 - 7) & (CELL_HS - 1);
  for (int probe = 0; probe < 24; ++probe) {
    const unsigned long long k = hk[s];
    if (k == key) return (int)s;
    if (k == EMPTY) return -1;
    s = (s + 1) & (CELL_HS - 1);
  }
  return -1;
}

struct CellLane {
  double qx, qy, qz, best, second;
  int bpos;
  unsigned int n_cand;
  bool ovf;
};

__device__ __forceinline__ bool cell_occupied(const GridView& g, int ix, int iy, int iz, BrickEntry& be, long long& last_b) {
  const long long b = ((long long)(iz >> 2) * g.by + (iy >> 2)) * g.bx + (ix >> 2);
  if (b != last_b) { be = g.bricks[b]; last_b = b; }
  return (be.mask >> ((ix & 3) | ((iy & 3) << 2) | ((iz & 3) << 4))) & 1ull;
}

__device__ __forceinline__ unsigned int cell_stage(const GridView& g, const unsigned long long* __restrict__ hk, unsigned int* __restrict__ hv,
                                                   unsigned int* __restrict__ hs, double* __restrict__ sx, double* __restrict__ sy, double* __restrict__ sz,
                                                   unsigned int* __restrict__ pool, int lane, unsigned int* n_pts) {
  unsigned int staged = 0;
  for (int s = lane; s < CELL_HS; s += 64) {
    const unsigned long long key = hk[s];
    if (key == EMPTY || hv[s] != CELL_UNSET) continue;
    const int ix = (int)(key & 0x1fffffull), iy = (int)((key >> 21) & 0x1fffffull), iz = (int)((key >> 42) & 0x1fffffull);
    const long long b = ((long long)(iz >> 2) * g.by + (iy >> 2)) * g.bx + (ix >> 2);
    const unsigned int tab = g.bricks[b].tab;
    const uint2 run = g.celltab[(size_t)tab * 64 + ((ix & 3) | ((iy & 3) << 2) | ((iz & 3) << 4))];
// ... 486 lines not shown
  MV_HIP(hipMemcpy(G.inv, G.h_inv.data(), sizeof(int) * (size_t)n, hipMemcpyHostToDevice));
  MV_HIP(hipMemcpy(G.table, table.data(), sizeof(HashEntry) * (size_t)tsize, hipMemcpyHostToDevice));
  G.struct_bytes = sizeof(HashEntry) * (double)tsize + sizeof(float) * 8.0 * nodes8;
  MV_CHECK(build_wide(f, spts.data()));
  MV_CHECK(build_mfma(f, spts.data()));
  f.has_grid = true;
  return MVICP_OK;
}

void free_grid(GridDev& g) {
  if (g.spts) (void)hipFree(g.spts);
  if (g.sidx) (void)hipFree(g.sidx);
  if (g.crec && g.crec != g.srec) (void)hipFree(g.crec);
  if (g.srec) (void)hipFree(g.srec);
  if (g.snor) (void)hipFree(g.snor);
  if (g.inv) (void)hipFree(g.inv);
  if (g.table) (void)hipFree(g.table);
  if (g.wide) (void)hipFree(g.wide);
  if (g.mf_ops) (void)hipFree(g.mf_ops);
  if (g.mf_blk) (void)hipFree(g.mf_blk);
  if (g.oct) (void)hipFree(g.oct);
  if (g.bricks) (void)hipFree(g.bricks);
  if (g.celltab) (void)hipFree(g.celltab);
  if (g.ov_samp) (void)hipFree(g.ov_samp);
  g = GridDev();
}

namespace {
GridView view_of(const FrameDev& f) {
  GridView v;
  const GridDev& g = f.grid;
  v.spts = g.spts; v.sidx = g.sidx; v.srec = (const PointRec*)g.srec; v.crec = (const PointRec*)g.crec; v.n = f.n;
  v.table = (const HashEntry*)g.table; v.mask = g.table_mask; v.shift = g.table_shift;
  v.ox = g.origin[0]; v.oy = g.origin[1]; v.oz = g.origin[2]; v.h = g.cell; v.inv_h = g.inv_cell;
  v.dx = g.dims[0]; v.dy = g.dims[1]; v.dz = g.dims[2];
  v.oct = g.oct; v.oct_leaf = g.oct_leaf; v.oct_first_leaf = g.oct_first_leaf;
  v.bricks = (const BrickEntry*)g.bricks; v.celltab = (const uint2*)g.celltab; v.bx = g.bdims[0]; v.by = g.bdims[1]; v.bz = g.bdims[2];
  return v;
}

int run(mvicp_ctx* c, std::vector<GridJob>& jobs, double bound, const FrameDev* const* dst_of, const SearchPlan* plan) {
  if (jobs.empty()) return MVICP_OK;
  const double search = search_bound(c, bound);
  std::vector<TieJob> ties;
  if (!(plan && plan->tie_skip)) {
    double launch_q = 0;
    for (const GridJob& j : jobs) launch_q += j.n;
    const TieRef tref = tie_ref(c, (size_t)launch_q, 0u);
    for (size_t k = 0; k < jobs.size(); ++k) {
      GridJob& j = jobs[k];
      j.tie = tref; j.tie.job = (unsigned int)k;
      TieJob t;
      std::memset(&t, 0, sizeof(t));
      tie_job_fill(*dst_of[k], t);
      t.q = j.q; t.xf = j.xf; t.n = j.n; t.out_idx = j.out_idx; t.out_d2 = j.out_d2; t.inv = j.inv; t.list = j.list;
      ties.push_back(t);
    }
  }
  int max_n = 0;
  double nq = 0;
  for (const GridJob& j : jobs) { max_n = std::max(max_n, j.n); nq += j.n; }
  if (max_n == 0) return MVICP_OK;
  GridJob* d_jobs = nullptr;
  MV_CHECK(cached_upload(c, jobs[0].xf ? "grid_jobs" : "grid_jobs_raw", jobs.data(), sizeof(GridJob) * jobs.size(), (void**)&d_jobs));
  unsigned long long* d_stats = nullptr;
  const size_t slots = (size_t)((max_n + NT - 1) / NT) * jobs.size() * (NT / 64);
  MV_CHECK(census_scratch(c, slots, &d_stats));
  const size_t total_q = (size_t)nq;
  if (total_q > c->far_cap) {
    if (c->d_far_list) MV_HIP(hipFree(c->d_far_list));
    MV_HIP(hipMalloc((void**)&c->d_far_list, sizeof(int2) * total_q));
    c->far_cap = total_q;
  }
  const bool edge_path = plan != nullptr;
  if (!c->d_far_count) {
    MV_HIP(hipMalloc((void**)&c->d_far_count, 2 * sizeof(unsigned int)));
    MV_HIP(hipMemsetAsync(c->d_far_count, 0, 2 * sizeof(unsigned int), c->stream));
    c->far_parity = 0;
  }
  unsigned int* far_cnt = c->d_far_count + c->far_parity;
  unsigned int* far_next = c->d_far_count + (c->far_parity ^ 1);
  c->far_parity ^= 1;
  bool use_cell = false;
  const dim3 grid((max_n + NT - 1) / NT, (unsigned)jobs.size());
  {
    ProfScope ps(c, "nn_grid", 36.0 * nq);
    use_cell = c->opt.nn_cell && !c->opt.nn_tree_only && !c->opt.nn_skip_far && edge_path;
    for (const GridJob& j : jobs) if (j.dst.bricks == nullptr || j.xf == nullptr) use_cell = false;
    std::snprintf(c->last_nn_launch, sizeof(c->last_nn_launch), "grid");
    if (c->opt.nn_tree_only)
      hipLaunchKernelGGL((nn_grid_kernel<true>), grid, dim3(NT), 0, c->stream, d_jobs, bound, search, d_stats, 0, (int2*)c->d_far_list, far_cnt, 0.0);
    else if (use_cell)
      hipLaunchKernelGGL(nn_cell_kernel, grid, dim3(NT), 0, c->stream, d_jobs, bound, search, d_stats, (int2*)c->d_far_list, far_cnt, c->prune_rho);
    else
      hipLaunchKernelGGL((nn_grid_kernel<false>), grid, dim3(NT), 0, c->stream, d_jobs, bound, search, d_stats, c->opt.nn_skip_far ? 1 : 0, (int2*)c->d_far_list, far_cnt,
                         c->prune_rho);
  }
  const bool launch_far = !(plan && plan->far_skip), launch_dirty = plan && !plan->nothing_can_change;
  if (launch_far || launch_dirty) {
    ProfScope ps(c, "nn_far", 0.0);
    const size_t far_wide = (plan && plan->far_narrow) ? 128 : 256 * 8;
    const unsigned int far_blocks = (unsigned int)std::min<size_t>(far_wide, (total_q * 8 + NT - 1) / NT);
    if (!c->h_far_seen) {
      MV_HIP(hipHostMalloc((void**)&c->h_far_seen, sizeof(unsigned int), hipHostMallocMapped));
      *c->h_far_seen = 1u;
      MV_HIP(hipHostGetDevicePointer((void**)&c->d_far_seen, c->h_far_seen, 0));
    }
    if (launch_far)
      hipLaunchKernelGGL(nn_far_kernel, dim3(far_blocks), dim3(NT), 0, c->stream, d_jobs, (const int2*)c->d_far_list, bound, (const unsigned int*)far_cnt, far_next, d_stats, slots,
                         edge_path ? c->d_far_seen : nullptr);
    if (launch_dirty)
      hipLaunchKernelGGL(dirty_reduce_kernel, dim3(c->E), dim3(256), 0, c->stream, c->E, c->d_dslot_off, c->d_dirty_slots, c->d_dirty);
  }
  MV_HIP(hipGetLastError());
  if (d_stats) MV_CHECK(census_collect(c, d_stats, slots, nq, c->opt.nn_tree_only ? 1 : (use_cell ? 3 : 0), "nn_grid"));
  MV_CHECK(launch_tie_fixup(c, ties, bound));
  return MVICP_OK;
}
}

int launch_dirty_reduce(mvicp_ctx* c) {
  hipLaunchKernelGGL(dirty_reduce_kernel, dim3(c->E), dim3(256), 0, c->stream, c->E, c->d_dslot_off, c->d_dirty_slots, c->d_dirty);
  MV_HIP(hipGetLastError());
  return MVICP_OK;
}

namespace { __global__ void grid_warm_kernel() {} }

int warm_nn_grid(mvicp_ctx* c) {
  if (!c->d_far_count) {
    MV_HIP(hipMalloc((void**)&c->d_far_count, 2 * sizeof(unsigned int)));
    MV_HIP(hipMemsetAsync(c->d_far_count, 0, 2 * sizeof(unsigned int), c->stream));
    c->far_parity = 0;
  }
  hipLaunchKernelGGL(grid_warm_kernel, dim3(1), dim3(64), 0, c->stream);
  MV_HIP(hipGetLastError());
  return MVICP_OK;
}

int launch_nn_grid_edges(mvicp_ctx* c, double d2_bound, const SearchPlan& plan) {
  std::vector<GridJob> jobs;
  std::vector<const FrameDev*> dsts;
  for (int e = 0; e < c->E; ++e) {
    if (!c->active[e]) continue;
    const FrameDev& s = c->frames[c->esrc[e]];
    const FrameDev& d = c->frames[c->edst[e]];
    if (!s.has_grid || !d.has_grid) { set_error("grid NN needs the per-cloud structure on frames %d and %d", c->esrc[e], c->edst[e]); return MVICP_ERR_STATE; }
    GridJob j;
    std::memset(&j, 0, sizeof(j));
    j.dst = view_of(d);
    j.q = s.grid.spts; j.qidx = nullptr; j.xf = c->d_xf + (size_t)e * kEdgeXf; j.n = s.n;
    j.out_idx = c->d_nn_idx + c->cap_off[e]; j.out_d2 = c->d_nn_d2 + c->cap_off[e];
    j.inv = d.grid.inv; j.out_lb = c->d_nn_lb + c->cap_off[e];
    j.list = ListRef{c->d_qpos + c->cap_off[e], c->d_second + c->cap_off[e], c->d_cd2 + c->cap_off[e], c->d_dirty + e, c->d_dirty_slots + c->dslot_off[e],
                     c->d_stream + c->cap_off[e], c->total_cap, d.grid.snor, (const PointRec*)d.grid.srec};
    j.seed = ((int)c->hist.nn_cache_edge.size() == c->E && c->hist.nn_cache_edge[e]) ? 1 : 0;
    jobs.push_back(j); dsts.push_back(&d);
  }
  return run(c, jobs, d2_bound, dsts.data(), &plan);
}

int launch_nn_grid_queries(mvicp_ctx* c, const FrameDev& f, const double* d_q, int n, int* d_idx, double* d_d2) {
  if (!f.has_grid) { set_error("grid NN structure missing"); return MVICP_ERR_STATE; }
  std::vector<GridJob> jobs(1);
  std::memset(&jobs[0], 0, sizeof(GridJob));
  jobs[0].dst = view_of(f);
  jobs[0].q = d_q; jobs[0].qidx = nullptr; jobs[0].xf = nullptr; jobs[0].n = n;
  jobs[0].out_idx = d_idx; jobs[0].out_d2 = d_d2;
  jobs[0].inv = nullptr; jobs[0].out_lb = nullptr;
  const FrameDev* dst = &f;
  return run(c, jobs, 1.7976931348623157e308, &dst, nullptr);
}

}
```

mv-lm-icp_amd/csrc/nn_list.h:

```cpp
#pragma once
#include "common.h"

namespace mvicp {

struct ListRef {
  const int* qpos; int* second; double* cd2; const int* dirty; int* dirty_slots;
  double* stream; long long total_cap; const double* dst_nor;
  const PointRec* dst_srec;
};

__device__ __forceinline__ void update_list_entry(const ListRef& R, int i, int idx_new, double d2_new, double bound, bool same_neighbour) {
  if (*R.dirty != 0) return;
  const int pos = R.qpos[i];
  const bool acc = idx_new >= 0 && d2_new < bound;
  bool clean;
  if (pos < 0) clean = !acc;
  else {
    clean = acc;
    if (clean) {
      if (!same_neighbour && R.second[pos] != idx_new) {
        R.second[pos] = idx_new;
        const double2* pb = reinterpret_cast<const double2*>(R.dst_srec + idx_new);
        const double2 b0 = pb[0], b1 = pb[1];
        double* st = R.stream + pos;
        st[7 * R.total_cap] = b0.x; st[8 * R.total_cap] = b0.y; st[9 * R.total_cap] = b1.x;
        if (R.dst_nor != nullptr) {
          const double n0 = R.dst_nor[3 * (size_t)idx_new], n1 = R.dst_nor[3 * (size_t)idx_new + 1], n2 = R.dst_nor[3 * (size_t)idx_new + 2];
          st[3 * R.total_cap] = n0; st[4 * R.total_cap] = n1; st[5 * R.total_cap] = n2;
          st[6 * R.total_cap] = n0 * b0.x + n1 * b0.y + n2 * b1.x;
        }
      }
      R.cd2[pos] = d2_new;
    }
  }
  if (!clean) R.dirty_slots[i / 256] = 1;
}

int launch_dirty_reduce(mvicp_ctx* c);

}
```

mv-lm-icp_amd/csrc/nn_tile_common.h:

```cpp
#pragma once
#include <algorithm>
#include <cmath>
#include <cstring>
#include <limits>
#include <vector>

#include "common.h"
#include "nn_cache.h"
#include "nn_census.h"
#include "nn_list.h"
#include "nn_metric.h"
#include "nn_tie.h"

namespace mvicp {

namespace {

constexpr int NT = 256;
#ifndef MVICP_TILE_LEAF
#define MVICP_TILE_LEAF 32
#endif
constexpr int LEAF = MVICP_TILE_LEAF;
constexpr int FAN = 64;

// ... 142 lines not shown
  const int lane = threadIdx.x & 63;
  const float inf = __int_as_float(0x7f800000);
  float b0 = inf, b1 = inf, b2 = inf, b3 = -inf, b4 = -inf, b5 = -inf;
  if (lane < nchild) {
    const float* base = g.wide + g.off[LEVEL] + first + lane;
    const long long st = g.cnt[LEVEL];
    b0 = base[0]; b1 = base[st]; b2 = base[2 * st]; b3 = base[3 * st]; b4 = base[4 * st]; b5 = base[5 * st];
  }
  return NodeBoxes{b0, b1, b2, b3, b4, b5};
}

__device__ __forceinline__ void node_cull(const PatchBox& G, const NodeBoxes& B, float& ddf, float& key) {
  const float e0 = fmaxf(fmaxf(B.b0 - G.hi[0], G.lo[0] - B.b3), 0.f);
  const float e1 = fmaxf(fmaxf(B.b1 - G.hi[1], G.lo[1] - B.b4), 0.f);
  const float e2 = fmaxf(fmaxf(B.b2 - G.hi[2], G.lo[2] - B.b5), 0.f);
  ddf = (e0 * e0 + e1 * e1 + e2 * e2) * 0.999999f;
  const float k0 = fmaxf(fmaxf(B.b0 - G.c[0], G.c[0] - B.b3), 0.f);
  const float k1 = fmaxf(fmaxf(B.b1 - G.c[1], G.c[1] - B.b4), 0.f);
  const float k2 = fmaxf(fmaxf(B.b2 - G.c[2], G.c[2] - B.b5), 0.f);
  key = k0 * k0 + k1 * k1 + k2 * k2;
}

__device__ __forceinline__ void node_park(float2* __restrict__ mybox, const NodeBoxes& B) {
  const int lane = threadIdx.x & 63;
  __builtin_amdgcn_wave_barrier();
  mybox[lane] = make_float2(B.b0, B.b3);
  mybox[FAN + lane] = make_float2(B.b1, B.b4);
  mybox[2 * FAN + lane] = make_float2(B.b2, B.b5);
  __builtin_amdgcn_fence(__ATOMIC_RELEASE, "wavefront");
  __builtin_amdgcn_wave_barrier();
  __builtin_amdgcn_fence(__ATOMIC_ACQUIRE, "wavefront");
}

template <bool IN_LDS>
__device__ __forceinline__ NodeBoxes node_child(const float2* __restrict__ mybox, const NodeBoxes& B, int c) {
  if (IN_LDS) {
    const float2 u = mybox[c], v = mybox[FAN + c], w = mybox[2 * FAN + c];
    return NodeBoxes{u.x, v.x, w.x, u.y, v.y, w.y};
  }
  return NodeBoxes{bcast(B.b0, c), bcast(B.b1, c), bcast(B.b2, c), bcast(B.b3, c), bcast(B.b4, c), bcast(B.b5, c)};
}

template <bool BND, bool BY_INDEX>
__device__ __forceinline__ void store_result(const TileJob& job, int i, int key, double best, double second, bool tie, float mu, double bound) {
  constexpr int NONE = BY_INDEX ? 0x7fffffff : -1;
  job.out_idx[i] = key == NONE ? -1 : (BY_INDEX && job.inv ? job.inv[key] : key);
  job.out_d2[i] = best;
  if (BND) job.out_lb[i] = key == NONE ? -1.f : __double2float_rd(fmin(sqrt(second), sqrt(best) + (double)mu) * (1.0 - 1e-9));
  if (job.list.dirty) update_list_entry(job.list, i, key == NONE ? -1 : (BY_INDEX ? job.inv[key] : key), best, bound, false);
  if ((BND ? second == best : tie) && key != NONE) tie_report(job.tie, (unsigned int)i);
}
TileView view_of(const FrameDev& f) {
  TileView v;
  v.spts = f.grid.spts; v.sidx = f.grid.sidx; v.n = f.n;
  v.wide = f.grid.wide; v.levels = f.grid.wide_levels;
  for (int l = 0; l < 6; ++l) { v.cnt[l] = f.grid.wide_cnt[l]; v.off[l] = f.grid.wide_off[l]; }
  v.maxabs = f.grid.maxabs;
  v.srec = (const PointRec*)f.grid.srec;
  v.mf_ops = (const uint4*)f.grid.mf_ops; v.mf_blk = (const MfBlock*)f.grid.mf_blk;
  return v;
}

inline int build_tile_jobs(mvicp_ctx* c, bool with_bounds, bool with_cache, bool with_list, std::vector<TileJob>& jobs, int& max_n, double& nq, std::vector<TieJob>& ties) {
  max_n = 0; nq = 0;
  double launch_q = 0;
  for (int e = 0; e < c->E; ++e) if (c->active[e]) launch_q += c->frames[c->esrc[e]].n;
  const TieRef tref = tie_ref(c, (size_t)launch_q, 0u);
  for (int e = 0; e < c->E; ++e) {
    if (!c->active[e]) continue;
    const FrameDev& s = c->frames[c->esrc[e]];
    const FrameDev& d = c->frames[c->edst[e]];
    if (!s.has_grid || !d.has_grid) { set_error("tile NN needs the per-cloud structure on frames %d and %d", c->esrc[e], c->edst[e]); return MVICP_ERR_STATE; }
    TileJob j;
    std::memset(&j, 0, sizeof(j));
    j.dst = view_of(d);
    j.q = s.grid.spts; j.qidx = nullptr; j.xf = c->d_xf + (size_t)e * kEdgeXf; j.n = s.n;
    j.out_idx = c->d_nn_idx + c->cap_off[e]; j.out_d2 = c->d_nn_d2 + c->cap_off[e];
    j.inv = d.grid.inv;
    j.seed = (c->tile_seed && (int)c->hist.nn_cache_edge.size() == c->E && c->hist.nn_cache_edge[e]) ? 1 : 0;
    if (with_bounds) { j.out_lb = c->d_nn_lb + c->cap_off[e]; j.mu = (float)(c->opt.tile_mu * d.grid.cell); }
    if (with_bounds && with_cache) { j.cache = 1; j.miss_max = c->tile_miss; j.reject_cache = c->reject_cache ? 1 : 0; }
    if (with_list) {
      j.list = ListRef{c->d_qpos + c->cap_off[e], c->d_second + c->cap_off[e], c->d_cd2 + c->cap_off[e], c->d_dirty + e, c->d_dirty_slots + c->dslot_off[e],
                       c->d_stream + c->cap_off[e], c->total_cap, d.grid.snor, (const PointRec*)d.grid.srec};
    }
    j.kacc = (float)c->mfma_kacc; j.trig = c->mfma_trig;
    j.tie = tref; j.tie.job = (unsigned int)jobs.size();
    {
      TieJob t;
      std::memset(&t, 0, sizeof(t));
      tie_job_fill(d, t);
      t.q = j.q; t.xf = j.xf; t.n = j.n; t.out_idx = j.out_idx; t.out_d2 = j.out_d2; t.inv = j.inv; t.list = j.list;
      ties.push_back(t);
    }
    jobs.push_back(j);
    max_n = std::max(max_n, s.n);
    nq += s.n;
  }
  return MVICP_OK;
}

template <typename Launch>
inline int launch_tile_search(mvicp_ctx* c, double d2_bound, bool with_bounds, bool with_cache, bool with_list, int wg, const char* scope, Launch launch) {
  std::vector<TileJob> jobs;
  int max_n = 0;
  double nq = 0;
  std::vector<TieJob> ties;
  MV_CHECK(build_tile_jobs(c, with_bounds, with_cache, with_list, jobs, max_n, nq, ties));
  if (jobs.empty() || max_n == 0) return MVICP_OK;
  TileJob* d_jobs = nullptr;
  MV_CHECK(cached_upload(c, jobs[0].xf ? "tile_jobs" : "tile_jobs_raw", jobs.data(), sizeof(TileJob) * jobs.size(), (void**)&d_jobs));
  unsigned long long* d_stats = nullptr;
  const size_t slots = (size_t)((max_n + wg - 1) / wg) * jobs.size() * (wg / 64);
  MV_CHECK(census_scratch(c, slots, &d_stats));
  {
    ProfScope ps(c, scope, 36.0 * nq);
    const dim3 grid((max_n + wg - 1) / wg, (unsigned)jobs.size());
    int top = jobs[0].dst.levels - 1;
    for (const TileJob& j : jobs) if (j.dst.levels - 1 != top) top = -1;
    launch(jobs, d_jobs, grid, top, d_stats);
  }
  MV_HIP(hipGetLastError());
  MV_CHECK(launch_tie_fixup(c, ties, d2_bound));
  if (with_list) MV_CHECK(launch_dirty_reduce(c));
  if (d_stats) MV_CHECK(census_collect(c, d_stats, slots, nq, 2, scope));
  return MVICP_OK;
}

}

}
```

mv-lm-icp_amd/csrc/search_plan.h:

```cpp
#pragma once
#include <algorithm>
#include <cmath>
#include <cstddef>
#include <cstring>
#include <limits>
#include <vector>

#include "../../include/mvicp.h"

namespace mvicp {

constexpr int kEdgeXf = 40;
constexpr int kXfRigid = 24;
constexpr int kXfCache = 24;
constexpr int kXfDM = 25;
constexpr int kXfDv = 34;
constexpr int kXfPad = 37;

inline double sqrt_bound(double t) {
  double x = t * t;
  while (std::sqrt(x) >= t && x > 0.0) x = std::nextafter(x, 0.0);
  while (std::sqrt(x) < t) x = std::nextafter(x, INFINITY);
  return x;
}

inline void inverse3(const double* m, double* r) {
#define M(i, j) m[(i) + 3 * (j)]
#define COF(i, j) (M(((i) + 1) % 3, ((j) + 1) % 3) * M(((i) + 2) % 3, ((j) + 2) % 3) - M(((i) + 1) % 3, ((j) + 2) % 3) * M(((i) + 2) % 3, ((j) + 1) % 3))
  const double c00 = COF(0, 0), c10 = COF(1, 0), c20 = COF(2, 0);
  const double det = (c00 * M(0, 0) + c10 * M(1, 0)) + c20 * M(2, 0);
  const double invdet = 1.0 / det;
  r[0] = c00 * invdet; r[3] = c10 * invdet; r[6] = c20 * invdet;
  r[1] = COF(0, 1) * invdet; r[4] = COF(1, 1) * invdet; r[7] = COF(2, 1) * invdet;
  r[2] = COF(0, 2) * invdet; r[5] = COF(1, 2) * invdet; r[8] = COF(2, 2) * invdet;
#undef COF
#undef M
}

inline void fill_query_xf(const double* Ps, const double* Pd, double* x) {
  double Rd[9];
  for (int j = 0; j < 3; ++j)
    for (int i = 0; i < 3; ++i) { x[i + 3 * j] = Ps[i + 4 * j]; Rd[i + 3 * j] = Pd[i + 4 * j]; }
  for (int i = 0; i < 3; ++i) { x[9 + i] = Ps[12 + i]; x[21 + i] = Pd[12 + i]; }
  inverse3(Rd, x + 12);
}

inline void query_affine(const double* x, double* Mq) {
  for (int j = 0; j < 3; ++j)
    for (int i = 0; i < 3; ++i) Mq[i + 3 * j] = x[12 + i] * x[0 + 3 * j] + x[12 + i + 3] * x[1 + 3 * j] + x[12 + i + 6] * x[2 + 3 * j];
  const double dt[3] = {x[9] - x[21], x[10] - x[22], x[11] - x[23]};
  for (int i = 0; i < 3; ++i) Mq[9 + i] = x[12 + i] * dt[0] + x[12 + i + 3] * dt[1] + x[12 + i + 6] * dt[2];
}

inline double cache_allowance_xf(const double* x_old, const double* x_new, double r) {
  if (std::memcmp(x_old, x_new, sizeof(double) * kXfRigid) == 0) return 0.0;
  double b = 0.0;
  for (const double* x : {x_old, x_new}) {
    double fr = 0.0, fi = 0.0;
    for (int k = 0; k < 9; ++k) { fr += x[k] * x[k]; fi += x[12 + k] * x[12 + k]; }
    const double dt[3] = {x[9] - x[21], x[10] - x[22], x[11] - x[23]};
    const double ts = std::sqrt(x[9] * x[9] + x[10] * x[10] + x[11] * x[11]), dtn = std::sqrt(dt[0] * dt[0] + dt[1] * dt[1] + dt[2] * dt[2]);
    b += std::sqrt(fi) * (ts + 16.0 * std::sqrt(fr) * r + 13.0 * dtn);
  }
  return std::max(0x1p-52 * b, std::numeric_limits<double>::min());
}

struct SearchOptions {
  bool list_reuse = true;
  bool nn_cache_enable = true;
  bool nn_tree_only = false;
  bool nn_skip_far = false;
  bool nn_cell = false;
  int tile_bounds = 1;
  int tile_cache = 1;
  int tile_mfma = 1;
  double cache_mfma_ratio = 3.0;
  double tile_mu = 0.02;
  bool sel_bracket = true;
  bool sel_reuse = true;
  bool spec_enable = true;
  bool spec2_enable = true;
  bool lin_pair = true;
  double auto_settle = 0.5;
  double auto_switch = 1.0;
  bool tie_rule = true;
  bool tie_lazy = true;
};

struct SearchHistory {
  bool have_corr = false;
  bool nn_cache_valid = false; float nn_cache_thresh = -1.f;
  std::vector<char> nn_cache_edge;
  std::vector<double> prev_q;
  std::vector<double> prev_xf;
  std::vector<char> list_valid;
  std::vector<char> explicit_list;
  std::vector<char> qpos_valid;
  std::vector<double> sel_med1, sel_med2;
  bool sel_result_valid = false;
  bool sel_result_armed = false;
  double auto_prev_dist = 0.0; int auto_last_method = -1;
  double last_rms = -1.0;
  unsigned int corr_tie_seen = 1u, corr_far_seen = 1u;
  bool prev_grid_kernel = false;
  bool spec_flags_valid = false; int spec_param = 0, spec_plane = 0, spec_robust = 0;
  std::vector<double> last_cand_poses;
  int last_cand_plane = -1, last_cand_robust = -1;
  std::vector<int> h_count;
  std::vector<float> h_weight;

  void forget(int E) {
    nn_cache_valid = false; nn_cache_thresh = -1.f;
    prev_q.assign((size_t)E * 12, 0.0); prev_xf.assign((size_t)E * kXfRigid, 0.0);
    nn_cache_edge.assign(E, 0);
    auto_prev_dist = 0.0; auto_last_method = -1; last_rms = -1.0; prev_grid_kernel = false;
    corr_tie_seen = corr_far_seen = 1u;
    list_valid.assign(E, 0);
    qpos_valid.assign(E, 0);
    sel_med1.assign(E, -1.0); sel_med2.assign(E, -1.0);
    sel_result_valid = false;
    spec_flags_valid = false;
    last_cand_poses.clear();
    have_corr = false;
    std::fill(h_count.begin(), h_count.end(), 0); std::fill(h_weight.begin(), h_weight.end(), 0.f);
  }
  void new_graph(int E) {
    h_count.assign(E, 0); h_weight.assign(E, 0.f); have_corr = false;
    sel_med1.assign(E, -1.0); sel_med2.assign(E, -1.0);
    nn_cache_valid = false; prev_q.assign((size_t)E * 12, 0.0); prev_xf.assign((size_t)E * kXfRigid, 0.0); nn_cache_edge.assign(E, 0);
    auto_prev_dist = 0.0; auto_last_method = -1; corr_tie_seen = corr_far_seen = 1u;
    list_valid.assign(E, 0); explicit_list.assign(E, 0); qpos_valid.assign(E, 0);
    sel_result_valid = false; sel_result_armed = false;
    last_cand_poses.clear();
  }
  void explicit_edge(int edge, int n, float weight) {
    nn_cache_valid = false;
    list_valid[edge] = 0; explicit_list[edge] = 1; qpos_valid[edge] = 0;
    sel_med1[edge] = sel_med2[edge] = -1.0;
    sel_result_valid = false;
    h_count[edge] = n; h_weight[edge] = weight;
    have_corr = true;
  }
};

struct PlanFrame { int n = 0; double max_norm = 0.0, cell = 0.0; bool has_grid = false, has_tie = false, has_snor = false; };
struct SearchInputs {
  int E = 0, n_frames = 0;
  const int* esrc = nullptr; const int* edst = nullptr; const char* owned = nullptr;
  const PlanFrame* frames = nullptr;
  const double* poses = nullptr; const unsigned char* fixed = nullptr;
  float thresh = 0.f; int nn_method = MVICP_NN_AUTO;
  bool exchange = false; int world = 1;
};

struct SearchPlan {
  char* active = nullptr;
  char* src_fixed = nullptr;
  double* xf = nullptr;
  int* nsrc = nullptr;
  int* dirty = nullptr;
  double* lohi = nullptr;
  std::vector<char> same_edge;
  std::vector<char> unchanged;
  std::vector<double> eps_ratio;
  std::vector<int> tie_need;
  bool all_same = true, same_active_set = false, all_unchanged = true;
  int method = MVICP_NN_TILE;
  bool tile_lb = false, tile_cached = false, handed_over = false;
  double eps_over_mu = -1.0;
  bool cached_on_mfma = false;
  bool nothing_can_change = false, tie_skip = false, far_skip = false, far_narrow = false, tie_launched = false, far_launched = false, sel_skip = false;
  bool use_bracket = false, spec_arm = false, spec2_plan = false;
  int status = MVICP_OK;
};

inline void plan_edges(const SearchInputs& in, const SearchOptions& opt, SearchHistory& h, SearchPlan& p) {
  const int E = in.E;
  const float thresh = in.thresh;
  const unsigned char* fixed = in.fixed;
  p.same_edge.assign(E, 0);
  p.unchanged.assign(E, 0);
  p.eps_ratio.clear();
  const bool hist_ok = h.have_corr && (int)h.nn_cache_edge.size() == E && h.nn_cache_thresh == thresh && (int)h.qpos_valid.size() == E;
  p.same_active_set = (int)h.nn_cache_edge.size() == E;
  for (int e = 0; e < E; ++e) {
    const PlanFrame& fs = in.frames[in.esrc[e]];
    const PlanFrame& fd = in.frames[in.edst[e]];
    p.active[e] = in.owned[e] && !(fixed && fixed[in.esrc[e]]);
    p.src_fixed[e] = fixed && fixed[in.esrc[e]];
    if (p.same_active_set && (p.active[e] != 0) != (h.nn_cache_edge[e] != 0)) p.same_active_set = false;
    p.nsrc[e] = p.active[e] ? fs.n : 0;
    double* x = p.xf + (size_t)e * kEdgeXf;
    fill_query_xf(in.poses + 16 * (size_t)in.esrc[e], in.poses + 16 * (size_t)in.edst[e], x);
    double Mq[12];
    query_affine(x, Mq);
    double* pq = &h.prev_q[(size_t)e * 12];
    for (int k = 0; k < 12; ++k) x[kXfDM + k] = Mq[k] - pq[k];
    const double rmax = fs.max_norm;
    if (p.active[e]) {
      double fro = 0.0;
      for (int k = 0; k < 9; ++k) fro += x[kXfDM + k] * x[kXfDM + k];
      const double eps_e = std::sqrt(fro) * rmax + std::sqrt(x[kXfDv] * x[kXfDv] + x[kXfDv + 1] * x[kXfDv + 1] + x[kXfDv + 2] * x[kXfDv + 2]);
      const double mu_e = opt.tile_mu * fd.cell;
      p.eps_ratio.push_back(mu_e > 0.0 ? eps_e / mu_e : 1e300);
    }
    const bool cache_on = h.nn_cache_valid && opt.nn_cache_enable && p.active[e] && (int)h.nn_cache_edge.size() == E && h.nn_cache_edge[e] &&
                          h.nn_cache_thresh == thresh;
    double* pxf = &h.prev_xf[(size_t)e * kXfRigid];
    const bool same_xf = std::memcmp(pxf, x, sizeof(double) * kXfRigid) == 0;
    if (!in.owned[e]) p.unchanged[e] = 1;
    else if (p.active[e]) p.unchanged[e] = hist_ok && h.nn_cache_edge[e] && h.qpos_valid[e] && !h.explicit_list[e] && same_xf;
    else p.unchanged[e] = hist_ok && !h.nn_cache_edge[e] && !h.explicit_list[e] && h.h_count[e] == 0;
    x[kXfCache] = cache_on ? cache_allowance_xf(pxf, x, rmax) : -1.0;
    p.same_edge[e] = cache_on && same_xf;
    std::memcpy(pxf, x, sizeof(double) * kXfRigid);
    for (int k = kXfPad; k < kEdgeXf; ++k) x[k] = 0.0;
    std::memcpy(pq, Mq, sizeof(Mq));
  }
  p.tie_need.clear();
  if (opt.tie_rule && !(opt.tie_lazy && in.world == 1))
    for (int e = 0; e < E; ++e) if (p.active[e] && !in.frames[in.edst[e]].has_tie) p.tie_need.push_back(in.edst[e]);
  p.all_same = true;
  for (int e = 0; e < E; ++e) if (p.active[e] && !p.same_edge[e]) p.all_same = false;
}

inline void choose_kernel(const SearchInputs& in, const SearchOptions& opt, SearchHistory& h, SearchPlan& p) {
  const int E = in.E;
  int method = in.nn_method;
  if (method == MVICP_NN_AUTO) {
    method = MVICP_NN_TILE;
    if (h.have_corr) {
      double dist = 0.0, cell = 0.0;
      int m = 0;
      for (int e = 0; e < E; ++e)
        if (h.h_count[e] > 0) { dist += h.h_weight[e] / 1.5; cell += in.frames[in.edst[e]].cell; ++m; }
      if (m > 0) {
        dist /= m; cell /= m;
        const bool settled = h.auto_prev_dist > 0.0 ? dist > opt.auto_settle * h.auto_prev_dist : dist < 0.5 * cell;
        if (opt.nn_cell) {
          double pred = dist;
          if (h.last_rms >= 0.0) pred = std::min(pred, std::sqrt(h.last_rms * h.last_rms + 0.09 * cell * cell));
          if (pred < opt.auto_switch * cell || h.auto_last_method == MVICP_NN_GRID) method = MVICP_NN_GRID;
        } else if (dist < 1.5 * cell && (settled || h.auto_last_method == MVICP_NN_GRID)) method = MVICP_NN_GRID;
        h.auto_prev_dist = dist;
      }
    }
  }
  if (method == MVICP_NN_GRID || method == MVICP_NN_TILE) {
    for (int e = 0; e < E; ++e)
      if (p.active[e] && (!in.frames[in.edst[e]].has_grid || !in.frames[in.esrc[e]].has_grid)) method = MVICP_NN_BRUTE;
  }
  const bool is_auto = in.nn_method == MVICP_NN_AUTO;
  p.tile_lb = false; p.handed_over = false;
  if (is_auto && method == MVICP_NN_GRID && h.auto_last_method == MVICP_NN_TILE && opt.tile_bounds >= 1 &&
      opt.nn_cache_enable && !opt.nn_cell) { method = MVICP_NN_TILE; p.tile_lb = true; p.handed_over = true; }
  if (method == MVICP_NN_TILE && opt.tile_bounds >= 2 && opt.nn_cache_enable) p.tile_lb = true;
  p.tile_cached = false;
  if (is_auto && method == MVICP_NN_GRID && !p.handed_over && opt.tile_cache && opt.tile_bounds >= 1 && h.nn_cache_valid &&
      opt.nn_cache_enable && !opt.nn_cell && !p.all_same) { method = MVICP_NN_TILE; p.tile_lb = true; p.tile_cached = true; p.handed_over = true; }
  if (method == MVICP_NN_TILE && !p.tile_cached && opt.tile_cache >= 2 && p.tile_lb && h.nn_cache_valid && opt.nn_cache_enable && !p.all_same) p.tile_cached = true;
  p.method = method;
  p.cached_on_mfma = false; p.eps_over_mu = -1.0;
  if (method == MVICP_NN_TILE && p.tile_cached && opt.tile_mfma == 1 && opt.cache_mfma_ratio > 0.0 && !p.eps_ratio.empty()) {
    std::nth_element(p.eps_ratio.begin(), p.eps_ratio.begin() + p.eps_ratio.size() / 2, p.eps_ratio.end());
    p.eps_over_mu = p.eps_ratio[p.eps_ratio.size() / 2];
    p.cached_on_mfma = p.eps_over_mu > opt.cache_mfma_ratio;
  }
}

inline void plan_search(const SearchInputs& in, const SearchOptions& opt, SearchHistory& h, SearchPlan& p) {
  const int E = in.E;
  plan_edges(in, opt, h, p);
  choose_kernel(in, opt, h, p);
  const int method = p.method;
  const bool is_auto = in.nn_method == MVICP_NN_AUTO;
  const bool grid_lists = method == MVICP_NN_GRID && !opt.nn_tree_only && !opt.nn_skip_far;
  const bool keep_lists = (method == MVICP_NN_TILE || grid_lists) && opt.list_reuse;
  for (int e = 0; e < E; ++e) p.dirty[e] = (keep_lists && p.active[e] && h.list_valid[e]) ? 0 : 1;
  p.use_bracket = opt.sel_bracket && h.have_corr;
  for (int e = 0; e < E; ++e) {
    p.lohi[2 * e] = p.lohi[2 * e + 1] = 0.0;
    if (!p.active[e]) continue;
    const double m1 = h.sel_med1[e], m2 = h.sel_med2[e];
    if (!(m1 > 0.0 && m2 > 0.0 && std::fabs(m1 - m2) <= 0.001 * m1)) { p.use_bracket = false; continue; }
    p.lohi[2 * e] = m1 * 0.994; p.lohi[2 * e + 1] = m1 * 1.006;
  }
  p.nothing_can_change = grid_lists && opt.list_reuse && p.same_active_set && !opt.nn_cell;
  for (int e = 0; e < E && p.nothing_can_change; ++e)
    if (p.active[e] && !(p.same_edge[e] && p.dirty[e] == 0)) p.nothing_can_change = false;
  p.tie_skip = p.nothing_can_change && h.corr_tie_seen == 0u;
  p.far_skip = p.nothing_can_change && h.corr_far_seen == 0u && h.prev_grid_kernel && method == MVICP_NN_GRID;
  p.tie_launched = opt.tie_rule && !p.tie_skip; p.far_launched = method == MVICP_NN_GRID && !p.far_skip;
  p.far_narrow = is_auto && method == MVICP_NN_GRID && h.nn_cache_valid && opt.nn_cache_enable && p.all_same;
  p.spec_arm = opt.spec_enable && h.spec_flags_valid;
  if (p.spec_arm && h.spec_plane)
    for (int e = 0; e < E; ++e) if (!p.src_fixed[e] && in.frames[in.edst[e]].n > 0 && !in.frames[in.edst[e]].has_snor) p.spec_arm = false;
  p.spec2_plan = p.spec_arm && !in.exchange && opt.spec2_enable && p.all_same && p.same_active_set && h.have_corr &&
                 h.last_cand_poses.size() == 16 * (size_t)in.n_frames && h.last_cand_plane == h.spec_plane && h.last_cand_robust == h.spec_robust;
  p.sel_skip = !in.exchange && opt.sel_reuse && p.nothing_can_change && h.sel_result_valid && (!p.spec_arm || h.sel_result_armed);
  p.status = (method != MVICP_NN_BRUTE && method != MVICP_NN_GRID && method != MVICP_NN_TILE) ? MVICP_ERR_ARG : MVICP_OK;
  p.all_unchanged = true;
  for (int e = 0; e < E; ++e) { if (!p.unchanged[e]) p.all_unchanged = false; if (p.status == MVICP_OK && p.active[e]) h.qpos_valid[e] = 0; }
}

inline void record_queued(const SearchInputs& in, const SearchOptions& opt, const SearchPlan& p, SearchHistory& h) {
  h.prev_grid_kernel = p.method == MVICP_NN_GRID;
  h.last_rms = -1.0;
  h.nn_cache_valid = ((p.method == MVICP_NN_GRID) && !opt.nn_tree_only && !opt.nn_skip_far) || p.tile_lb;
  h.nn_cache_thresh = in.thresh;
  h.auto_last_method = p.handed_over ? MVICP_NN_GRID : p.method;
  h.nn_cache_edge.assign(p.active, p.active + in.E);
  for (int e = 0; e < in.E; ++e) { h.list_valid[e] = p.active[e]; if (in.owned[e]) h.qpos_valid[e] = p.active[e]; if (p.active[e]) h.explicit_list[e] = 0; }
}

inline bool record_arrived(const SearchInputs& in, const SearchPlan& p, SearchHistory& h, unsigned int tie_word, unsigned int far_word, const double* res,
                           const double* scales, bool redone) {
  const int E = in.E;
  if (p.tie_launched) h.corr_tie_seen = tie_word;
  if (p.far_launched) h.corr_far_seen = far_word;
  else if (p.method != MVICP_NN_GRID) h.corr_far_seen = 1u;
  bool spec_bad = redone;
  if (p.spec_arm && res[2 * (size_t)E] != (double)(in.exchange ? in.world : 1)) spec_bad = true;
  for (int e = 0; e < E; ++e) {
    const bool mine = in.owned[e] && p.active[e];
    const double cnt = (in.exchange || mine) ? res[2 * e] : 0.0, med = cnt > 0 ? res[2 * e + 1] : 0.0;
    if (!mine) h.sel_med1[e] = h.sel_med2[e] = -1.0;
    else { h.sel_med2[e] = h.sel_med1[e]; h.sel_med1[e] = cnt > 0 ? med : -1.0; }
    if (p.spec_arm && !spec_bad && (in.exchange || mine)) {
      const double a_host = cnt > 0 ? (double)(float)(std::sqrt(med) * 1.5) : 0.0;
      if (scales[e] != a_host) spec_bad = true;
    }
    h.h_count[e] = (int)cnt;
    h.h_weight[e] = h.h_count[e] > 0 ? (float)(std::sqrt(med) * 1.5) : 0.f;
  }
  if (!p.sel_skip) h.sel_result_armed = p.spec_arm;
  h.sel_result_valid = !in.exchange;
  h.have_corr = true;
  return p.spec_arm && !spec_bad;
}

}
```

mv-lm-icp_amd/mvicp/lib.py:

```python
import ctypes as C
import os

import numpy as np

_HERE = os.path.dirname(os.path.abspath(__file__))
LIB_PATH = os.environ.get("MVICP_LIB") or os.path.join(os.path.dirname(_HERE), "libmvicp_hip.so")

PARAM_EIGEN_QUATERNION, PARAM_ANGLE_AXIS, PARAM_SOPHUS_SE3 = 0, 1, 2
METRIC_POINT, METRIC_PLANE, METRIC_SYMMETRIC = 0, 1, 2
NN_AUTO, NN_BRUTE, NN_GRID, NN_TILE = 0, 1, 2, 3
ORIENT_ANCHOR, ORIENT_VIEWPOINT, ORIENT_DIRECTION = 0, 1, 2
EDGE_BLOCK = 91

SYMBOLS = [
    "mvicp_last_error", "mvicp_version", "mvicp_create", "mvicp_destroy", "mvicp_set_num_frames", "mvicp_set_frame",
    "mvicp_recompute_normals", "mvicp_set_graph", "mvicp_set_shard", "mvicp_edge_owner", "mvicp_comm_unique_id", "mvicp_comm_init", "mvicp_comm_nranks", "mvicp_comm_set_callback", "mvicp_correspond",
    "mvicp_get_correspondences", "mvicp_map_correspondences", "mvicp_map_correspondences_async", "mvicp_wait_correspondences", "mvicp_correspondence_epochs", "mvicp_set_correspondences", "mvicp_nn_query", "mvicp_linearize", "mvicp_linearize_pair", "mvicp_linearize_metric", "mvicp_linearize_gicp", "mvicp_optimize", "mvicp_optimize_metric", "mvicp_optimize_gicp",
    "mvicp_lm_solve", "mvicp_set_option", "mvicp_nn_census", "mvicp_nn_census_ex", "mvicp_last_nn_launch", "mvicp_reset_history", "mvicp_profile_enable", "mvicp_profile_reset", "mvicp_profile_get", "mvicp_profile_get_ex", "mvicp_stream", "mvicp_sync",
    "mvicp_closedform_point_to_point", "mvicp_closedform_point_to_plane", "mvicp_set_frame_device", "mvicp_get_structure",
    "mvicp_overlap", "mvicp_graph_from_overlap", "mvicp_voxel_grid", "mvicp_voxel_fetch",
    "mvicp_outlier_filter", "mvicp_outlier_fetch", "mvicp_outlier_threshold", "mvicp_cache_allowance",
    "mvicp_knn_search", "mvicp_knn_fetch", "mvicp_fpfh", "mvicp_fpfh_fetch", "mvicp_iss_keypoints", "mvicp_iss_fetch",
    "mvicp_estimate_normals", "mvicp_normals_fetch", "mvicp_normals_adopt", "mvicp_fit_normals", "mvicp_normals_fit_fetch",
    "mvicp_orient_normals", "mvicp_orient_fetch", "mvicp_orient_adopt", "mvicp_normal_agreement", "mvicp_signs_from_agreement", "mvicp_negate_normals",
    "mvicp_feature_match", "mvicp_feature_match_fetch", "mvicp_match_pairs", "mvicp_consensus", "mvicp_consensus_fetch",
    "mvicp_coarse_pairs", "mvicp_coarse_pairs_fetch", "mvicp_poses_from_pairs",
]

STRUCTURE_NAMES = ("spts", "sidx", "srec", "crec", "inv", "snor", "table", "oct", "wide", "mf_ops", "mf_blk", "bricks", "celltab",
                   "h_order", "h_inv", "scalars")


class MvicpError(RuntimeError):
    pass


class Summary(C.Structure):
    _fields_ = [("initial_cost", C.c_double), ("final_cost", C.c_double), ("iterations", C.c_int), ("successful_steps", C.c_int),
                ("termination", C.c_int), ("evaluations", C.c_int)]

    def as_dict(self):
        return {k: getattr(self, k) for k, _ in self._fields_}


class OutlierStats(C.Structure):
    _fields_ = [("n", C.c_longlong), ("kept", C.c_longlong), ("q_exp", C.c_int), ("has_normals", C.c_int), ("s1", C.c_ulonglong),
                ("s2_hi", C.c_ulonglong), ("s2_lo", C.c_ulonglong), ("T", C.c_double), ("threshold", C.c_double)]

    def as_dict(self):
        d = {k: getattr(self, k) for k, _ in self._fields_}
        d["s2"] = (d["s2_hi"] << 64) | d["s2_lo"]
        return d


class ConsensusResult(C.Structure):
    _fields_ = [("best", C.c_int), ("count", C.c_int), ("accepted", C.c_int), ("reserved", C.c_int), ("pose", C.c_double * 16)]


class CoarseEdge(C.Structure):
    _fields_ = [("pairs", C.c_int), ("best", C.c_int), ("count", C.c_int), ("accepted", C.c_int), ("pose", C.c_double * 16)]


ALLREDUCE_FN = C.CFUNCTYPE(C.c_int, C.c_void_p, C.POINTER(C.c_double), C.c_size_t)
EVAL_FN = C.CFUNCTYPE(C.c_int, C.c_void_p, C.POINTER(C.c_double), C.POINTER(C.c_double))

_lib = None


def load_library(path=None):
    global _lib
    if _lib is not None and path is None:
        return _lib
    p = path or LIB_PATH
    if not os.path.exists(p):
        raise MvicpError(f"{p} not found: build it with `make -C mv-lm-icp_amd` (or __graft_entry__.build())")
    lib = C.CDLL(p, mode=C.RTLD_GLOBAL)
    vp, ip, dp, fp, u8p = C.c_void_p, C.POINTER(C.c_int), C.POINTER(C.c_double), C.POINTER(C.c_float), C.POINTER(C.c_ubyte)
    lib.mvicp_last_error.restype = C.c_char_p
    lib.mvicp_version.restype = C.c_char_p
    lib.mvicp_create.argtypes = [C.c_int, C.POINTER(vp)]
    lib.mvicp_destroy.argtypes = [vp]
    lib.mvicp_set_num_frames.argtypes = [vp, C.c_int]
    lib.mvicp_set_frame.argtypes = [vp, C.c_int, dp, dp, C.c_int]
    lib.mvicp_recompute_normals.argtypes = [vp, C.c_int, C.c_int, dp, ip]
    lib.mvicp_set_graph.argtypes = [vp, C.c_int, ip, ip]
    lib.mvicp_set_shard.argtypes = [vp, C.c_int, C.c_int]
    lib.mvicp_edge_owner.argtypes = [C.c_int, ip, C.c_int, ip]
    lib.mvicp_comm_unique_id.argtypes = [C.c_char_p, vp]
    lib.mvicp_comm_init.argtypes = [vp, C.c_char_p, vp, C.c_int, C.c_int]
    lib.mvicp_comm_set_callback.argtypes = [vp, ALLREDUCE_FN, vp]
    lib.mvicp_comm_nranks.argtypes = [vp]
    lib.mvicp_correspond.argtypes = [vp, dp, u8p, C.c_float, C.c_int, ip, fp]
    lib.mvicp_get_correspondences.argtypes = [vp, C.c_int, C.c_int, ip, ip, dp]
    lib.mvicp_map_correspondences.argtypes = [vp, C.POINTER(vp), C.POINTER(C.POINTER(C.c_longlong))]
    lib.mvicp_map_correspondences_async.argtypes = [vp, C.POINTER(vp), C.POINTER(C.POINTER(C.c_longlong))]
    lib.mvicp_wait_correspondences.argtypes = [vp, C.c_int]
    lib.mvicp_correspondence_epochs.argtypes = [vp, C.POINTER(C.POINTER(C.c_ulonglong))]
    lib.mvicp_set_correspondences.argtypes = [vp, C.c_int, C.c_int, ip, ip, C.c_float]
    lib.mvicp_nn_query.argtypes = [vp, C.c_int, dp, C.c_int, C.c_int, ip, dp]
    lib.mvicp_linearize.argtypes = [vp, dp, C.c_int, C.c_int, dp]
    lib.mvicp_linearize_pair.argtypes = [vp, dp, dp, C.c_int, C.c_int, dp, dp]
    lib.mvicp_optimize.argtypes = [vp, dp, u8p, C.c_int, C.c_int, C.c_int, C.c_int, C.POINTER(Summary)]
    lib.mvicp_linearize_metric.argtypes = [vp, dp, C.c_int, C.c_int, dp]
    lib.mvicp_optimize_metric.argtypes = [vp, dp, u8p, C.c_int, C.c_int, C.c_int, C.c_int, C.POINTER(Summary)]
    lib.mvicp_linearize_gicp.argtypes = [vp, dp, C.c_double, C.c_int, dp]
    lib.mvicp_optimize_gicp.argtypes = [vp, dp, u8p, C.c_int, C.c_double, C.c_int, C.c_int, C.POINTER(Summary)]
    lib.mvicp_lm_solve.argtypes = [C.c_int, C.c_int, ip, ip, dp, u8p, C.c_int, C.c_int, EVAL_FN, vp, C.POINTER(Summary)]
    lib.mvicp_set_option.argtypes = [vp, C.c_char_p, C.c_double]
    lib.mvicp_nn_census.argtypes = [vp, dp]
    lib.mvicp_nn_census_ex.argtypes = [vp, dp, C.c_int]
    lib.mvicp_last_nn_launch.argtypes = [vp]
    lib.mvicp_last_nn_launch.restype = C.c_char_p
    lib.mvicp_reset_history.argtypes = [vp]
    lib.mvicp_profile_enable.argtypes = [vp, C.c_int]
    lib.mvicp_profile_reset.argtypes = [vp]
    lib.mvicp_profile_get.argtypes = [vp, C.c_char_p, dp, C.POINTER(C.c_longlong), dp]
    lib.mvicp_profile_get_ex.argtypes = [vp, C.c_char_p, dp, C.c_int]
    lib.mvicp_stream.argtypes = [vp]
    lib.mvicp_stream.restype = vp
    lib.mvicp_sync.argtypes = [vp]
    lib.mvicp_closedform_point_to_point.argtypes = [dp, dp, C.c_int, dp]
    lib.mvicp_closedform_point_to_plane.argtypes = [dp, dp, dp, C.c_int, dp]
    lib.mvicp_set_frame_device.argtypes = [vp, C.c_int, vp, vp, C.c_int]
    lib.mvicp_get_structure.argtypes = [vp, C.c_int, C.c_char_p, vp, C.c_longlong]
    lib.mvicp_get_structure.restype = C.c_longlong
    llp = C.POINTER(C.c_longlong)
    lib.mvicp_overlap.argtypes = [vp, dp, C.c_float, C.c_int, ip, ip, llp, ip]
    lib.mvicp_graph_from_overlap.argtypes = [C.c_int, ip, ip, llp, C.c_int, C.c_double, C.c_int, C.c_int, ip, ip, ip]
    lib.mvicp_voxel_grid.argtypes = [vp, C.c_int, ip, dp, C.c_double, ip]
    lib.mvicp_voxel_grid.restype = C.c_longlong
    lib.mvicp_voxel_fetch.argtypes = [vp, C.c_longlong, vp, vp, vp]
    lib.mvicp_outlier_filter.argtypes = [vp, C.c_int, C.c_int, C.c_double, C.c_double, C.POINTER(OutlierStats)]
    lib.mvicp_outlier_filter.restype = C.c_longlong
    lib.mvicp_outlier_fetch.argtypes = [vp, C.c_longlong, vp, vp, vp, C.c_longlong, vp, vp]
    lib.mvicp_outlier_threshold.argtypes = [C.c_longlong, C.c_ulonglong, C.c_ulonglong, C.c_ulonglong, C.c_double, dp]
    lib.mvicp_cache_allowance.argtypes = [dp, dp, dp, dp, C.c_double, dp]
    lib.mvicp_knn_search.argtypes = [vp, C.c_int, vp, C.c_longlong, C.c_int, C.c_double]
    lib.mvicp_knn_search.restype = C.c_longlong
    lib.mvicp_knn_fetch.argtypes = [vp, C.c_longlong, C.c_longlong, vp, vp, vp, vp]
    lib.mvicp_fpfh.argtypes = [vp, C.c_int, C.c_double, C.c_int]
    lib.mvicp_fpfh.restype = C.c_longlong
    lib.mvicp_fpfh_fetch.argtypes = [vp, C.c_longlong, vp, vp]
    lib.mvicp_iss_keypoints.argtypes = [vp, C.c_int, C.c_double, C.c_double, C.c_double, C.c_double, C.c_int]
    lib.mvicp_iss_keypoints.restype = C.c_longlong
    lib.mvicp_iss_fetch.argtypes = [vp, C.c_longlong, vp, vp, vp, C.c_longlong, vp, vp, vp]
    lib.mvicp_estimate_normals.argtypes = [vp, C.c_int, C.c_int, C.c_double, dp]
    lib.mvicp_estimate_normals.restype = C.c_longlong
    lib.mvicp_normals_fetch.argtypes = [vp, C.c_longlong, vp, vp, vp]
    lib.mvicp_normals_adopt.argtypes = [vp]
    lib.mvicp_fit_normals.argtypes = [vp, C.c_int, C.c_int, C.c_double, dp, C.c_int]
    lib.mvicp_fit_normals.restype = C.c_longlong
    lib.mvicp_normals_fit_fetch.argtypes = [vp, C.c_longlong, vp]
    lib.mvicp_orient_normals.argtypes = [vp, C.c_int, C.c_int, C.c_int, C.c_double, C.c_int, dp]
    lib.mvicp_orient_normals.restype = C.c_longlong
    lib.mvicp_orient_fetch.argtypes = [vp, C.c_longlong, vp, vp, vp]
    lib.mvicp_orient_adopt.argtypes = [vp]
    lib.mvicp_normal_agreement.argtypes = [vp, dp, ip, ip]
    lib.mvicp_signs_from_agreement.argtypes = [C.c_int, C.c_int, ip, ip, ip, ip, C.c_int, C.POINTER(C.c_ubyte), ip]
    lib.mvicp_negate_normals.argtypes = [vp, C.c_int]
    lib.mvicp_feature_match.argtypes = [vp, vp, C.c_longlong, vp, C.c_longlong, C.c_int]
    lib.mvicp_feature_match.restype = C.c_longlong
    lib.mvicp_feature_match_fetch.argtypes = [vp, C.c_longlong, C.c_longlong, vp, vp, vp, vp]
    lib.mvicp_match_pairs.argtypes = [C.c_longlong, C.c_longlong, vp, vp, vp, C.c_int, C.c_double, vp]
    lib.mvicp_match_pairs.restype = C.c_longlong
    lib.mvicp_consensus.argtypes = [vp, vp, vp, C.c_longlong, C.c_longlong, C.c_ulonglong, C.c_double, C.c_double, C.POINTER(ConsensusResult)]
    lib.mvicp_consensus_fetch.argtypes = [vp, C.c_longlong, vp, C.c_longlong, vp]
    lib.mvicp_coarse_pairs.argtypes = [vp, vp, vp, llp, C.c_int, C.c_int, C.c_int, ip, ip, C.POINTER(C.c_ulonglong), C.c_int, C.c_double,
                                       C.c_longlong, C.c_double, C.c_double, C.POINTER(CoarseEdge)]
    lib.mvicp_coarse_pairs.restype = C.c_longlong
    lib.mvicp_coarse_pairs_fetch.argtypes = [vp, C.c_int, C.c_longlong, vp, vp]
    lib.mvicp_poses_from_pairs.argtypes = [C.c_int, C.c_int, ip, ip, ip, dp, C.c_int, C.c_int, dp, dp, ip, ip, ip]
    if path is None:
        _lib = lib
    return lib


def _dp(a):
    return a.ctypes.data_as(C.POINTER(C.c_double))


# ... 371 lines not shown
        _check(self.lib, self.lib.mvicp_comm_set_callback(self.h, self._ar_cb, None))

    @staticmethod
    def comm_unique_id(librccl_path=None):
        lib = load_library()
        buf = (C.c_char * 128)()
        path = librccl_path.encode() if librccl_path else None
        _check(lib, lib.mvicp_comm_unique_id(path, C.cast(buf, C.c_void_p)))
        return bytes(buf)

    def _round_buffers(self, K):
        b = getattr(self, "_rb", None)
        if b is None or b["K"] != K or b["E"] != self.E:
            P = np.zeros((K, 16)); fx = np.zeros(K, dtype=np.uint8)
            counts = np.zeros(self.E, dtype=np.int32); weights = np.zeros(self.E, dtype=np.float32)
            sm = Summary()
            b = {"K": K, "E": self.E, "P": P, "P44": P.reshape(K, 4, 4), "fx": fx, "counts": counts, "weights": weights, "sm": sm,
                 "pP": _dp(P), "pfx": fx.ctypes.data_as(C.POINTER(C.c_ubyte)), "pc": _ip(counts), "pw": weights.ctypes.data_as(C.POINTER(C.c_float)),
                 "psm": C.byref(sm)}
            self._rb = b
        return b

    def correspond(self, poses, fixed, thresh, nn_method=NN_AUTO):
        b = self._round_buffers(len(poses))
        np.copyto(b["P44"], np.transpose(np.asarray(poses, dtype=np.float64), (0, 2, 1)))
        b["fx"][:] = fixed
        _check(self.lib, self.lib.mvicp_correspond(self.h, b["pP"], b["pfx"], np.float32(thresh), nn_method, b["pc"], b["pw"]))
        self.counts = b["counts"].copy()
        return self.counts, b["weights"].copy()

    def round_state(self, K, fixed):
        b = self._round_buffers(K)
        b["fx"][:] = fixed
        return b

    def correspond_raw(self, thresh, nn_method=NN_AUTO):
        b = self._rb
        _check(self.lib, self.lib.mvicp_correspond(self.h, b["pP"], b["pfx"], thresh, nn_method, b["pc"], b["pw"]))

    def optimize_raw(self, param, point_to_plane, robust, max_iterations=50):
        b = self._rb
        _check(self.lib, self.lib.mvicp_optimize(self.h, b["pP"], b["pfx"], param, int(point_to_plane), int(robust), max_iterations, b["psm"]))
        return b["sm"]

    def get_correspondences(self, edge):
        cap = self.npts[self.src[edge]]
        first = np.zeros(cap, dtype=np.int32)
        second = np.zeros(cap, dtype=np.int32)
        dist = np.zeros(cap, dtype=np.float64)
        n = _check(self.lib, self.lib.mvicp_get_correspondences(self.h, edge, cap, _ip(first), _ip(second), _dp(dist)))
        return first[:n].copy(), second[:n].copy(), dist[:n].copy()

    CORR_DTYPE = np.dtype([("first", np.int32), ("second", np.int32), ("dist", np.float64)])

    def map_correspondences(self, copy=True):
        tp, op = C.c_void_p(), C.POINTER(C.c_longlong)()
        _check(self.lib, self.lib.mvicp_map_correspondences(self.h, C.byref(tp), C.byref(op)))
        off = np.ctypeslib.as_array(op, shape=(self.E + 1,)).copy()
        total = int(off[-1])
        if total == 0:
            return np.zeros(0, dtype=self.CORR_DTYPE), off
        buf = (C.c_char * (16 * total)).from_address(tp.value)
        t = np.frombuffer(buf, dtype=self.CORR_DTYPE, count=total)
        return (t.copy() if copy else t), off

    def map_correspondences_async(self):
        tp, op = C.c_void_p(), C.POINTER(C.c_longlong)()
        _check(self.lib, self.lib.mvicp_map_correspondences_async(self.h, C.byref(tp), C.byref(op)))
        off = np.ctypeslib.as_array(op, shape=(self.E + 1,)).copy()
        total = int(off[-1])
        if total == 0:
            return np.zeros(0, dtype=self.CORR_DTYPE), off
        buf = (C.c_char * (16 * total)).from_address(tp.value)
        return np.frombuffer(buf, dtype=self.CORR_DTYPE, count=total), off

    def wait_correspondences(self, edge):
        _check(self.lib, self.lib.mvicp_wait_correspondences(self.h, int(edge)))

    def correspondence_epochs(self):
        ep = C.POINTER(C.c_ulonglong)()
        _check(self.lib, self.lib.mvicp_correspondence_epochs(self.h, C.byref(ep)))
        return np.ctypeslib.as_array(ep, shape=(self.E,)).copy()

    def set_correspondences(self, edge, first, second, weight=0.0):
        first = np.ascontiguousarray(first, dtype=np.int32)
        second = np.ascontiguousarray(second, dtype=np.int32)
        _check(self.lib, self.lib.mvicp_set_correspondences(self.h, edge, len(first), _ip(first), _ip(second), np.float32(weight)))

    def overlap(self, poses, thresh, max_samples=4096):
        P = poses_to_c(poses)
        K = len(P)
        samples = np.zeros(K, dtype=np.int32); hits = np.zeros((K, K), dtype=np.int32); sumq = np.zeros((K, K), dtype=np.int64)
        q = C.c_int(0)
        _check(self.lib, self.lib.mvicp_overlap(self.h, _dp(P), np.float32(thresh), int(max_samples), _ip(samples), _ip(hits),
                                                sumq.ctypes.data_as(C.POINTER(C.c_longlong)), C.byref(q)))
        fraction = hits / np.maximum(samples, 1)[:, None].astype(np.float64)
        mean_d2 = np.ldexp(sumq / np.maximum(hits, 1).astype(np.float64), -q.value)
        return {"samples": samples, "hits": hits, "sumq": sumq, "q_exp": int(q.value), "fraction": fraction, "mean_d2": mean_d2}

    def _result_arrays(self, device):
        if device:
            import torch
            dev = torch.device("cuda", self.device)
            return (lambda shape, dt: torch.empty(shape, dtype=dt, device=dev),
                    lambda t: C.c_void_p(t.data_ptr()) if t is not None and t.numel() else None,
                    lambda: torch.cuda.synchronize(dev), torch.float64, torch.int32, torch.int64, torch.uint8)
        return (lambda shape, dt: np.zeros(shape, dtype=dt),
                lambda a: a.ctypes.data_as(C.c_void_p) if a is not None and a.size else None,
                lambda: None, np.float64, np.int32, np.int64, np.uint8)

    def voxel_grid(self, voxel, frames=None, poses=None, device=False):
        if frames is None:
            n_sel, fp = 0, None
        else:
            fr = np.ascontiguousarray(frames, dtype=np.int32).reshape(-1)
            n_sel = len(fr)
            fr = np.concatenate([fr, np.zeros(1, dtype=np.int32)])
            fp = _ip(fr)
        P = None if poses is None else poses_to_c(poses)
        hn = C.c_int(0)
        st = self.lib.mvicp_voxel_grid(self.h, n_sel, fp, _dp(P) if P is not None else None, float(voxel), C.byref(hn))
        m = int(_check(self.lib, st))
        has_nrm = bool(hn.value)
        mk, ptr, ready, f64, i32, i64, u8 = self._result_arrays(device)
        xyz, nrm, cnt = mk((m, 3), f64), (mk((m, 3), f64) if has_nrm else None), mk((m,), i32)
        ready()
        _check(self.lib, self.lib.mvicp_voxel_fetch(self.h, m, ptr(xyz), ptr(nrm), ptr(cnt)))
        return {"xyz": xyz, "nrm": nrm, "cnt": cnt}

    def outlier_filter(self, frame, k=16, std_ratio=2.0, radius=0.0, device=False):
        S = OutlierStats()
        kept = int(_check(self.lib, self.lib.mvicp_outlier_filter(self.h, int(frame), int(k), float(std_ratio), float(radius), C.byref(S))))
        n = int(S.n)
        has_nrm = bool(S.has_normals)
        mk, ptr, ready, f64, i32, i64, u8 = self._result_arrays(device)
        xyz, nrm, idx = mk((kept, 3), f64), (mk((kept, 3), f64) if has_nrm else None), mk((kept,), i32)
        mdist, kd2 = mk((n,), f64), mk((n,), f64)
        ready()
        _check(self.lib, self.lib.mvicp_outlier_fetch(self.h, kept, ptr(xyz), ptr(nrm), ptr(idx), n, ptr(mdist), ptr(kd2)))
        return {"xyz": xyz, "nrm": nrm, "idx": idx, "mdist": mdist, "kd2": kd2, "stats": S.as_dict()}

    def knn_search(self, frame, queries=None, k=8, radius=0.0, device=False):
        keep = None
        if queries is None:
            qp, m = None, 0
        elif isinstance(queries, np.ndarray) or not hasattr(queries, "data_ptr"):
            keep = np.ascontiguousarray(queries, dtype=np.float64).reshape(-1, 3)
            m = len(keep)
            qp = keep.ctypes.data_as(C.c_void_p) if m else C.cast(C.create_string_buffer(24), C.c_void_p)
        else:
            import torch
            if not queries.is_cuda or queries.dtype != torch.float64 or (queries.device.index or 0) != self.device:
                raise MvicpError("knn_search: a torch `queries` must be a float64 tensor on the engine's GPU")
            keep = queries.contiguous().reshape(-1, 3)
            m = keep.shape[0]
            torch.cuda.synchronize(keep.device)
            qp = C.c_void_p(keep.data_ptr()) if m else C.cast(C.create_string_buffer(24), C.c_void_p)
        total = int(_check(self.lib, self.lib.mvicp_knn_search(self.h, int(frame), qp, m, int(k), float(radius))))
        if queries is None:
            m = self.npts[int(frame)]
        k = int(k)
        entries = m * k if k else total
        mk, ptr, ready, f64, i32, i64, u8 = self._result_arrays(device)
        cnt, off, idx, d2 = mk((m,), i32), mk((m + 1,), i64), mk((entries,), i32), mk((entries,), f64)
        ready()
        _check(self.lib, self.lib.mvicp_knn_fetch(self.h, m, entries, ptr(cnt), ptr(off), ptr(idx), ptr(d2)))
# ... 246 lines not shown
```

Baseline: 1185 iterations/s.

## Build correspondence lists directly during NN search for fresh edges

Edges whose lists are invalid but not the same edge as before are marked fresh. The grid NN kernel then writes the correspondence list entries and the linearization stream operands in place, indexed by query, instead of relying on a separate list rebuild. If every query is accepted, the dirty reduce kernel promotes the list to kept and sets the count, so the rebuild pass is skipped. A new list-origin API reports how each list was produced. The cost is a templated kernel variant with extra writes per query and an identity-ordered list layout.

```diff
diff --git a/include/mvicp.h b/include/mvicp.h
--- a/include/mvicp.h
+++ b/include/mvicp.h
@@ -139,6 +139,8 @@
 int mvicp_correspond(mvicp_ctx* ctx, const double* poses, const unsigned char* fixed, float thresh, int nn_method,
                      int* counts, float* weights);
 int mvicp_reset_history(mvicp_ctx* ctx);
+enum { MVICP_LIST_KEPT = 0, MVICP_LIST_REBUILT = 1, MVICP_LIST_BUILT_BY_SEARCH = 2 };
+int mvicp_list_origin(mvicp_ctx* ctx, const int** origin);
 int mvicp_get_correspondences(mvicp_ctx* ctx, int edge, int cap, int* first, int* second, double* dist);
 typedef struct mvicp_corr { int first; int second; double dist; } mvicp_corr;
 int mvicp_map_correspondences(mvicp_ctx* ctx, const mvicp_corr** triples, const long long** offsets);
diff --git a/mv-lm-icp_amd/csrc/api.cpp b/mv-lm-icp_amd/csrc/api.cpp
--- a/mv-lm-icp_amd/csrc/api.cpp
+++ b/mv-lm-icp_amd/csrc/api.cpp
@@ -150,7 +150,7 @@
   dev_free(c->d_chunk_first); dev_free(c->d_partials); dev_free(c->d_out);
   c->sym_lo_pin.release(); c->sym_lo_dev.release();
   if (c->h_pin) (void)hipHostFree(c->h_pin);
-  c->h_pin = nullptr; c->h_pin_doubles = 0; c->d_res_host = nullptr; c->d_blocks_host = nullptr; c->lin_out = nullptr;
+  c->h_pin = nullptr; c->h_pin_doubles = 0; c->h_list_origin = nullptr; c->d_list_origin = nullptr; c->d_res_host = nullptr; c->d_blocks_host = nullptr; c->lin_out = nullptr;
   c->census_pending = false; c->spec_ready = false; c->spec2_ready = false; c->spec_arm = false; c->d_spec_host = nullptr; c->d_adev_host = nullptr; c->d_res_target = nullptr; c->d_a_check = nullptr;
   dev_free(c->d_xblock_cnt); c->export_valid = false; c->export_in_flight = false; c->export_chunks = 0;
   for (hipEvent_t ev : c->export_events) (void)hipEventDestroy(ev);
@@ -1564,6 +1564,9 @@
     MV_HIP(hipHostGetDevicePointer(&dp, c->h_pin, 0));
     c->d_blocks_host = (double*)dp + c->pin_blocks_off;
     c->d_res_host = (double*)dp + c->pin_res_off;
+    c->h_list_origin = reinterpret_cast<int*>(c->h_pin + c->pin_misc_off);
+    c->d_list_origin = reinterpret_cast<int*>((double*)dp + c->pin_misc_off);
+    for (int e = 0; e < E; ++e) c->h_list_origin[e] = MVICP_LIST_REBUILT;
     c->d_spec_host = (double*)dp + c->pin_spec_off;
     c->d_adev_host = (double*)dp + c->pin_adev_off;
     c->d_spec2_host = (double*)dp + c->pin_spec2_off;
@@ -1649,6 +1652,13 @@
 }
 
 static int launch_local_search(mvicp_ctx* c, const SearchInputs& in, const SearchPlan& plan, double bound, size_t upload_doubles, CorrMarks& mark) {
+  {
+    int* h_dirty = reinterpret_cast<int*>(c->h_pin + (size_t)c->E * kEdgeXf) + c->E;
+    for (int e = 0; e < c->E; ++e) {
+      c->h_list_origin[e] = h_dirty[e] != 0 ? MVICP_LIST_REBUILT : MVICP_LIST_KEPT;
+      if (plan.fresh[e]) h_dirty[e] = kListFresh;
+    }
+  }
   MV_HIP(hipMemcpyAsync(c->d_ctl, c->h_pin, sizeof(double) * upload_doubles, hipMemcpyHostToDevice, c->stream));
   if (c->fault_inject > 0 && --c->fault_inject == 0) { set_error("injected launch failure (option fault_inject)"); return MVICP_ERR_HIP; }
   if (plan.method == MVICP_NN_BRUTE) MV_CHECK(launch_nn_brute_edges(c));
@@ -1851,6 +1861,15 @@
   return MVICP_OK;
 } MVICP_GUARD_ABI
 
+int mvicp_list_origin(mvicp_ctx* c, const int** origin) try {
+  MV_CHECK(bind(c));
+  if (!origin) { set_error("null output"); return MVICP_ERR_ARG; }
+  if (c->E == 0) { set_error("no graph"); return MVICP_ERR_STATE; }
+  if (!c->hist.have_corr) { set_error("no correspondences yet"); return MVICP_ERR_STATE; }
+  *origin = c->h_list_origin;
+  return MVICP_OK;
+} MVICP_GUARD_ABI
+
 int mvicp_correspondence_epochs(mvicp_ctx* c, const unsigned long long** epochs) try {
   MV_CHECK(bind(c));
   if (!epochs) { set_error("null output"); return MVICP_ERR_ARG; }
@@ -2025,6 +2044,7 @@
   if (std::strcmp(name, "nn_cache") == 0) { c->opt.nn_cache_enable = value != 0.0; c->hist.nn_cache_valid = false; return MVICP_OK; }
   if (std::strcmp(name, "lin_chunk") == 0) { c->lin_chunk_override = (int)value; return MVICP_OK; }
   if (std::strcmp(name, "list_reuse") == 0) { c->opt.list_reuse = value != 0.0; return MVICP_OK; }
+  if (std::strcmp(name, "first_lists") == 0) { c->opt.first_lists = value != 0.0; return MVICP_OK; }
   if (std::strcmp(name, "lin_interleave") == 0) { c->lin_interleave = value != 0.0; return MVICP_OK; }
   if (std::strcmp(name, "lin_share_p") == 0) { c->lin_share_p = value != 0.0; return MVICP_OK; }
   if (std::strcmp(name, "lin_pair") == 0) { c->opt.lin_pair = value != 0.0; return MVICP_OK; }
diff --git a/mv-lm-icp_amd/csrc/common.h b/mv-lm-icp_amd/csrc/common.h
--- a/mv-lm-icp_amd/csrc/common.h
+++ b/mv-lm-icp_amd/csrc/common.h
@@ -235,6 +235,7 @@
   int* d_first = nullptr; int* d_second = nullptr; double* d_cd2 = nullptr;
   int* d_qpos = nullptr;
   int* d_dirty = nullptr;
+  int* h_list_origin = nullptr; int* d_list_origin = nullptr;
   int* d_dirty_slots = nullptr; int* d_dslot_off = nullptr; std::vector<int> dslot_off; int n_dslots = 0;
   void* d_export = nullptr; void* h_export = nullptr; size_t export_cap = 0;
   int* d_xblock_cnt = nullptr;
diff --git a/mv-lm-icp_amd/csrc/nn_cache.h b/mv-lm-icp_amd/csrc/nn_cache.h
--- a/mv-lm-icp_amd/csrc/nn_cache.h
+++ b/mv-lm-icp_amd/csrc/nn_cache.h
@@ -19,12 +19,12 @@
 
 __device__ __forceinline__ bool cache_still_none(double allowance, const float* out_lb, int i) { return allowance == 0.0 && out_lb[i] == -1.f; }
 
-template <typename Job>
+template <typename Job, bool FRESH = true>
 __device__ __forceinline__ void cache_refresh(const Job& job, int i, int pi, double d, double eps, float lb_old, double bound) {
   if (eps != 0.0) {
     job.out_d2[i] = d;
     job.out_lb[i] = __double2float_rd((double)lb_old - eps);
-    if (job.list.dirty) update_list_entry(job.list, i, pi, d, bound, true);
+    if (job.list.dirty) update_list_entry<FRESH>(job.list, i, pi, d, bound, true);
   }
 }
 
diff --git a/mv-lm-icp_amd/csrc/nn_grid.hip b/mv-lm-icp_amd/csrc/nn_grid.hip
--- a/mv-lm-icp_amd/csrc/nn_grid.hip
+++ b/mv-lm-icp_amd/csrc/nn_grid.hip
@@ -36,17 +36,17 @@
   const BrickEntry* bricks; const uint2* celltab; int bx, by, bz;
 };
 
-struct GridJob {
+struct alignas(64) GridJob {
   GridView dst;
   const double* q; const int* qidx;
   const double* xf;
   int n;
   int* out_idx; double* out_d2;
   const int* inv;
-  ListRef list;
   float* out_lb;
   int seed;
   TieRef tie;
+  ListRef list;
 };
 
 __device__ __forceinline__ unsigned long long __reduce_add_u64(unsigned long long v) {
@@ -64,17 +64,23 @@
   return (int)(threadIdx.x & 63) == __ffsll((long long)mask) - 1;
 }
 
-__global__ void dirty_reduce_kernel(int E, const int* __restrict__ slot_off, int* __restrict__ slots, int* __restrict__ dirty) {
+__global__ void dirty_reduce_kernel(int E, const int* __restrict__ slot_off, int* __restrict__ slots, int* __restrict__ dirty,
+                                    const int* __restrict__ nsrc, int* __restrict__ count, int* __restrict__ origin) {
   const int e = blockIdx.x;
   int any = 0;
   for (int k = slot_off[e] + threadIdx.x; k < slot_off[e + 1]; k += blockDim.x) {
     const int v = slots[k];
     if (v) { any = 1; slots[k] = 0; }
   }
-  if (__syncthreads_or(any) && threadIdx.x == 0) dirty[e] = 1;
-}
-
-template <bool TREE_ONLY>
+  any = __syncthreads_or(any);
+  if (threadIdx.x != 0) return;
+  const int was = dirty[e];
+  if (any) dirty[e] = kListDirty;
+  else if (was == kListFresh) { dirty[e] = kListKeep; count[e] = nsrc[e]; }
+  origin[e] = (any || was == kListDirty) ? MVICP_LIST_REBUILT : was == kListFresh ? MVICP_LIST_BUILT_BY_SEARCH : MVICP_LIST_KEPT;
+}
+
+template <bool TREE_ONLY, bool FRESH>
 __global__ __launch_bounds__(NT) void nn_grid_kernel(const GridJob* __restrict__ jobs, double bound, double search, unsigned long long* __restrict__ stats, int skip_far,
                                                      int2* __restrict__ far_list, unsigned int* __restrict__ far_count, double prune_rho) {
   __shared__ double sxf[kEdgeXf];
@@ -122,7 +128,7 @@
         const double eps = cache_eps(sxf, p0, p1, p2);
         const float lb_old = job.out_lb[out];
         if (cache_hit(eps, lb_old, d, bound, true, false)) {
-          cache_refresh(job, out, pi, d, eps, lb_old, bound);
+          cache_refresh<GridJob, FRESH>(job, out, pi, d, eps, lb_old, bound);
           if (stats) {
             unsigned long long c1 = __reduce_add_u64(1ull);
             const size_t slot = ((size_t)blockIdx.y * gridDim.x + blockIdx.x) * (NT / 64) + (threadIdx.x >> 6);
@@ -214,7 +220,7 @@
   job.out_idx[out] = bi == 0x7fffffff ? -1 : (job.inv ? job.inv[bi] : bi);
   job.out_d2[out] = best;
   if (job.out_lb != nullptr) job.out_lb[out] = resolved ? __double2float_rd(sqrt(fmin(fmin(second, m2), skipped)) * (1.0 - 1e-12)) : 0.f;
-  if (job.list.dirty && (resolved || skip_far)) update_list_entry(job.list, i, bi == 0x7fffffff ? -1 : job.inv[bi], best, bound, false);
+  if (job.list.dirty && (resolved || skip_far)) update_list_entry<FRESH>(job.list, i, bi == 0x7fffffff ? -1 : job.inv[bi], best, bound, false);
   if (resolved && bi != 0x7fffffff && second == best) tie_report(job.tie, (unsigned int)i);
   if (!resolved && !skip_far) {
     const unsigned long long mask = __ballot(1);
@@ -867,6 +873,8 @@
   unsigned int* far_next = c->d_far_count + (c->far_parity ^ 1);
   c->far_parity ^= 1;
   bool use_cell = false;
+  bool any_fresh = false;
+  if (plan) for (char f : plan->fresh) any_fresh = any_fresh || f != 0;
   const dim3 grid((max_n + NT - 1) / NT, (unsigned)jobs.size());
   {
     ProfScope ps(c, "nn_grid", 36.0 * nq);
@@ -874,11 +882,14 @@
     for (const GridJob& j : jobs) if (j.dst.bricks == nullptr || j.xf == nullptr) use_cell = false;
     std::snprintf(c->last_nn_launch, sizeof(c->last_nn_launch), "grid");
     if (c->opt.nn_tree_only)
-      hipLaunchKernelGGL((nn_grid_kernel<true>), grid, dim3(NT), 0, c->stream, d_jobs, bound, search, d_stats, 0, (int2*)c->d_far_list, far_cnt, 0.0);
+      hipLaunchKernelGGL((nn_grid_kernel<true, false>), grid, dim3(NT), 0, c->stream, d_jobs, bound, search, d_stats, 0, (int2*)c->d_far_list, far_cnt, 0.0);
     else if (use_cell)
       hipLaunchKernelGGL(nn_cell_kernel, grid, dim3(NT), 0, c->stream, d_jobs, bound, search, d_stats, (int2*)c->d_far_list, far_cnt, c->prune_rho);
+    else if (any_fresh)
+      hipLaunchKernelGGL((nn_grid_kernel<false, true>), grid, dim3(NT), 0, c->stream, d_jobs, bound, search, d_stats, c->opt.nn_skip_far ? 1 : 0, (int2*)c->d_far_list, far_cnt,
+                         c->prune_rho);
     else
-      hipLaunchKernelGGL((nn_grid_kernel<false>), grid, dim3(NT), 0, c->stream, d_jobs, bound, search, d_stats, c->opt.nn_skip_far ? 1 : 0, (int2*)c->d_far_list, far_cnt,
+      hipLaunchKernelGGL((nn_grid_kernel<false, false>), grid, dim3(NT), 0, c->stream, d_jobs, bound, search, d_stats, c->opt.nn_skip_far ? 1 : 0, (int2*)c->d_far_list, far_cnt,
                          c->prune_rho);
   }
   const bool launch_far = !(plan && plan->far_skip), launch_dirty = plan && !plan->nothing_can_change;
@@ -895,7 +906,8 @@
       hipLaunchKernelGGL(nn_far_kernel, dim3(far_blocks), dim3(NT), 0, c->stream, d_jobs, (const int2*)c->d_far_list, bound, (const unsigned int*)far_cnt, far_next, d_stats, slots,
                          edge_path ? c->d_far_seen : nullptr);
     if (launch_dirty)
-      hipLaunchKernelGGL(dirty_reduce_kernel, dim3(c->E), dim3(256), 0, c->stream, c->E, c->d_dslot_off, c->d_dirty_slots, c->d_dirty);
+      hipLaunchKernelGGL(dirty_reduce_kernel, dim3(c->E), dim3(256), 0, c->stream, c->E, c->d_dslot_off, c->d_dirty_slots, c->d_dirty,
+                         (const int*)c->d_nsrc, c->d_count, c->d_list_origin);
   }
   MV_HIP(hipGetLastError());
   if (d_stats) MV_CHECK(census_collect(c, d_stats, slots, nq, c->opt.nn_tree_only ? 1 : (use_cell ? 3 : 0), "nn_grid"));
@@ -905,7 +917,8 @@
 }
 
 int launch_dirty_reduce(mvicp_ctx* c) {
-  hipLaunchKernelGGL(dirty_reduce_kernel, dim3(c->E), dim3(256), 0, c->stream, c->E, c->d_dslot_off, c->d_dirty_slots, c->d_dirty);
+  hipLaunchKernelGGL(dirty_reduce_kernel, dim3(c->E), dim3(256), 0, c->stream, c->E, c->d_dslot_off, c->d_dirty_slots, c->d_dirty,
+                         (const int*)c->d_nsrc, c->d_count, c->d_list_origin);
   MV_HIP(hipGetLastError());
   return MVICP_OK;
 }
@@ -938,7 +951,7 @@
     j.out_idx = c->d_nn_idx + c->cap_off[e]; j.out_d2 = c->d_nn_d2 + c->cap_off[e];
     j.inv = d.grid.inv; j.out_lb = c->d_nn_lb + c->cap_off[e];
     j.list = ListRef{c->d_qpos + c->cap_off[e], c->d_second + c->cap_off[e], c->d_cd2 + c->cap_off[e], c->d_dirty + e, c->d_dirty_slots + c->dslot_off[e],
-                     c->d_stream + c->cap_off[e], c->total_cap, d.grid.snor, (const PointRec*)d.grid.srec};
+                     c->d_stream + c->cap_off[e], c->total_cap, d.grid.snor, (const PointRec*)d.grid.srec, (const PointRec*)s.grid.srec, c->d_first + c->cap_off[e]};
     j.seed = ((int)c->hist.nn_cache_edge.size() == c->E && c->hist.nn_cache_edge[e]) ? 1 : 0;
     jobs.push_back(j); dsts.push_back(&d);
   }
diff --git a/mv-lm-icp_amd/csrc/nn_list.h b/mv-lm-icp_amd/csrc/nn_list.h
--- a/mv-lm-icp_amd/csrc/nn_list.h
+++ b/mv-lm-icp_amd/csrc/nn_list.h
@@ -3,16 +3,43 @@
 
 namespace mvicp {
 
+constexpr int kListKeep = 0, kListDirty = 1, kListFresh = 2;
+
 struct ListRef {
-  const int* qpos; int* second; double* cd2; const int* dirty; int* dirty_slots;
+  int* qpos; int* second; double* cd2; const int* dirty; int* dirty_slots;
   double* stream; long long total_cap; const double* dst_nor;
   const PointRec* dst_srec;
+  const PointRec* src_srec; int* first;
 };
 
+__device__ __forceinline__ void write_target_operands(const ListRef& R, int pos, int idx_new) {
+  const double2* pb = reinterpret_cast<const double2*>(R.dst_srec + idx_new);
+  const double2 b0 = pb[0], b1 = pb[1];
+  double* st = R.stream + pos;
+  st[7 * R.total_cap] = b0.x; st[8 * R.total_cap] = b0.y; st[9 * R.total_cap] = b1.x;
+  if (R.dst_nor != nullptr) {
+    const double n0 = R.dst_nor[3 * (size_t)idx_new], n1 = R.dst_nor[3 * (size_t)idx_new + 1], n2 = R.dst_nor[3 * (size_t)idx_new + 2];
+    st[3 * R.total_cap] = n0; st[4 * R.total_cap] = n1; st[5 * R.total_cap] = n2;
+    st[6 * R.total_cap] = n0 * b0.x + n1 * b0.y + n2 * b1.x;
+  }
+}
+
+template <bool FRESH = true>
 __device__ __forceinline__ void update_list_entry(const ListRef& R, int i, int idx_new, double d2_new, double bound, bool same_neighbour) {
-  if (*R.dirty != 0) return;
+  const int state = *R.dirty;
+  if (FRESH ? state == kListDirty : state != kListKeep) return;
+  const bool acc = idx_new >= 0 && d2_new < bound;
+  if (FRESH && state == kListFresh) {
+    if (!acc) { R.dirty_slots[i / 256] = 1; return; }
+    R.qpos[i] = i; R.first[i] = i; R.second[i] = idx_new; R.cd2[i] = d2_new;
+    const double2* pa = reinterpret_cast<const double2*>(R.src_srec + i);
+    const double2 a0 = pa[0], a1 = pa[1];
+    double* st = R.stream + i;
+    st[0] = a0.x; st[R.total_cap] = a0.y; st[2 * R.total_cap] = a1.x;
+    write_target_operands(R, i, idx_new);
+    return;
+  }
   const int pos = R.qpos[i];
-  const bool acc = idx_new >= 0 && d2_new < bound;
   bool clean;
   if (pos < 0) clean = !acc;
   else {
@@ -20,15 +47,7 @@
     if (clean) {
       if (!same_neighbour && R.second[pos] != idx_new) {
         R.second[pos] = idx_new;
-        const double2* pb = reinterpret_cast<const double2*>(R.dst_srec + idx_new);
-        const double2 b0 = pb[0], b1 = pb[1];
-        double* st = R.stream + pos;
-        st[7 * R.total_cap] = b0.x; st[8 * R.total_cap] = b0.y; st[9 * R.total_cap] = b1.x;
-        if (R.dst_nor != nullptr) {
-          const double n0 = R.dst_nor[3 * (size_t)idx_new], n1 = R.dst_nor[3 * (size_t)idx_new + 1], n2 = R.dst_nor[3 * (size_t)idx_new + 2];
-          st[3 * R.total_cap] = n0; st[4 * R.total_cap] = n1; st[5 * R.total_cap] = n2;
-          st[6 * R.total_cap] = n0 * b0.x + n1 * b0.y + n2 * b1.x;
-        }
+        write_target_operands(R, pos, idx_new);
       }
       R.cd2[pos] = d2_new;
     }
diff --git a/mv-lm-icp_amd/csrc/nn_tile_common.h b/mv-lm-icp_amd/csrc/nn_tile_common.h
--- a/mv-lm-icp_amd/csrc/nn_tile_common.h
+++ b/mv-lm-icp_amd/csrc/nn_tile_common.h
@@ -248,7 +248,7 @@
     if (with_bounds && with_cache) { j.cache = 1; j.miss_max = c->tile_miss; j.reject_cache = c->reject_cache ? 1 : 0; }
     if (with_list) {
       j.list = ListRef{c->d_qpos + c->cap_off[e], c->d_second + c->cap_off[e], c->d_cd2 + c->cap_off[e], c->d_dirty + e, c->d_dirty_slots + c->dslot_off[e],
-                       c->d_stream + c->cap_off[e], c->total_cap, d.grid.snor, (const PointRec*)d.grid.srec};
+                       c->d_stream + c->cap_off[e], c->total_cap, d.grid.snor, (const PointRec*)d.grid.srec, (const PointRec*)s.grid.srec, c->d_first + c->cap_off[e]};
     }
     j.kacc = (float)c->mfma_kacc; j.trig = c->mfma_trig;
     j.tie = tref; j.tie.job = (unsigned int)jobs.size();
diff --git a/mv-lm-icp_amd/csrc/search_plan.h b/mv-lm-icp_amd/csrc/search_plan.h
--- a/mv-lm-icp_amd/csrc/search_plan.h
+++ b/mv-lm-icp_amd/csrc/search_plan.h
@@ -67,6 +67,7 @@
 
 struct SearchOptions {
   bool list_reuse = true;
+  bool first_lists = true;
   bool nn_cache_enable = true;
   bool nn_tree_only = false;
   bool nn_skip_far = false;
@@ -162,6 +163,7 @@
   double* lohi = nullptr;
   std::vector<char> same_edge;
   std::vector<char> unchanged;
+  std::vector<char> fresh;
   std::vector<double> eps_ratio;
   std::vector<int> tie_need;
   bool all_same = true, same_active_set = false, all_unchanged = true;
@@ -277,6 +279,8 @@
   const bool grid_lists = method == MVICP_NN_GRID && !opt.nn_tree_only && !opt.nn_skip_far;
   const bool keep_lists = (method == MVICP_NN_TILE || grid_lists) && opt.list_reuse;
   for (int e = 0; e < E; ++e) p.dirty[e] = (keep_lists && p.active[e] && h.list_valid[e]) ? 0 : 1;
+  p.fresh.assign(E, 0);
+  for (int e = 0; e < E; ++e) p.fresh[e] = keep_lists && opt.first_lists && p.active[e] && p.dirty[e] != 0 && !p.same_edge[e];
   p.use_bracket = opt.sel_bracket && h.have_corr;
   for (int e = 0; e < E; ++e) {
     p.lohi[2 * e] = p.lohi[2 * e + 1] = 0.0;
diff --git a/mv-lm-icp_amd/mvicp/lib.py b/mv-lm-icp_amd/mvicp/lib.py
--- a/mv-lm-icp_amd/mvicp/lib.py
+++ b/mv-lm-icp_amd/mvicp/lib.py
@@ -11,11 +11,12 @@
 NN_AUTO, NN_BRUTE, NN_GRID, NN_TILE = 0, 1, 2, 3
 ORIENT_ANCHOR, ORIENT_VIEWPOINT, ORIENT_DIRECTION = 0, 1, 2
 EDGE_BLOCK = 91
+LIST_KEPT, LIST_REBUILT, LIST_BUILT_BY_SEARCH = 0, 1, 2
 
 SYMBOLS = [
     "mvicp_last_error", "mvicp_version", "mvicp_create", "mvicp_destroy", "mvicp_set_num_frames", "mvicp_set_frame",
     "mvicp_recompute_normals", "mvicp_set_graph", "mvicp_set_shard", "mvicp_edge_owner", "mvicp_comm_unique_id", "mvicp_comm_init", "mvicp_comm_nranks", "mvicp_comm_set_callback", "mvicp_correspond",
-    "mvicp_get_correspondences", "mvicp_map_correspondences", "mvicp_map_correspondences_async", "mvicp_wait_correspondences", "mvicp_correspondence_epochs", "mvicp_set_correspondences", "mvicp_nn_query", "mvicp_linearize", "mvicp_linearize_pair", "mvicp_linearize_metric", "mvicp_linearize_gicp", "mvicp_optimize", "mvicp_optimize_metric", "mvicp_optimize_gicp",
+    "mvicp_get_correspondences", "mvicp_map_correspondences", "mvicp_map_correspondences_async", "mvicp_wait_correspondences", "mvicp_correspondence_epochs", "mvicp_list_origin", "mvicp_set_correspondences", "mvicp_nn_query", "mvicp_linearize", "mvicp_linearize_pair", "mvicp_linearize_metric", "mvicp_linearize_gicp", "mvicp_optimize", "mvicp_optimize_metric", "mvicp_optimize_gicp",
     "mvicp_lm_solve", "mvicp_set_option", "mvicp_nn_census", "mvicp_nn_census_ex", "mvicp_last_nn_launch", "mvicp_reset_history", "mvicp_profile_enable", "mvicp_profile_reset", "mvicp_profile_get", "mvicp_profile_get_ex", "mvicp_stream", "mvicp_sync",
     "mvicp_closedform_point_to_point", "mvicp_closedform_point_to_plane", "mvicp_set_frame_device", "mvicp_get_structure",
     "mvicp_overlap", "mvicp_graph_from_overlap", "mvicp_voxel_grid", "mvicp_voxel_fetch",
@@ -96,6 +97,7 @@
     lib.mvicp_map_correspondences_async.argtypes = [vp, C.POINTER(vp), C.POINTER(C.POINTER(C.c_longlong))]
     lib.mvicp_wait_correspondences.argtypes = [vp, C.c_int]
     lib.mvicp_correspondence_epochs.argtypes = [vp, C.POINTER(C.POINTER(C.c_ulonglong))]
+    lib.mvicp_list_origin.argtypes = [vp, C.POINTER(C.POINTER(C.c_int))]
     lib.mvicp_set_correspondences.argtypes = [vp, C.c_int, C.c_int, ip, ip, C.c_float]
     lib.mvicp_nn_query.argtypes = [vp, C.c_int, dp, C.c_int, C.c_int, ip, dp]
     lib.mvicp_linearize.argtypes = [vp, dp, C.c_int, C.c_int, dp]
@@ -633,6 +635,11 @@
         _check(self.lib, self.lib.mvicp_correspondence_epochs(self.h, C.byref(ep)))
         return np.ctypeslib.as_array(ep, shape=(self.E,)).copy()
 
+    def list_origin(self):
+        op = C.POINTER(C.c_int)()
+        _check(self.lib, self.lib.mvicp_list_origin(self.h, C.byref(op)))
+        return np.ctypeslib.as_array(op, shape=(self.E,)).copy()
+
     def set_correspondences(self, edge, first, second, weight=0.0):
         first = np.ascontiguousarray(first, dtype=np.int32)
         second = np.ascontiguousarray(second, dtype=np.int32)
```

Measured after the change: 1197 iterations/s (median of 6 runs). About the same (+1.0%).
